# wecacuee/Bayesian_CBF

Hardware: AMD Instinct MI355X
Metric: control steps/sec (GP posterior + CBF-QP) at N_train=512, batch=4096; HBM GB/s vs peak (higher is better)
Workload: dtype f32

## Files before the change

### bayesian_cbf_amd/_lib.py

```python
import ctypes
import os

import torch

_HERE = os.path.dirname(os.path.abspath(__file__))
LIB_PATH = os.environ.get("BCBF_LIB_PATH") or os.path.join(_HERE, "libbcbf.so")

c_int, c_void_p, c_size_t = ctypes.c_int, ctypes.c_void_p, ctypes.c_size_t
c_float, c_double = ctypes.c_float, ctypes.c_double
P = c_void_p

_SIGS = {
    "bcbf_version": (c_int, []),
    "bcbf_last_error": (ctypes.c_char_p, []),
    "bcbf_hbm_read_probe": (c_int, [P, c_size_t, P, ctypes.POINTER(c_size_t), P]),
    "bcbf_lop_elems_f32": (c_size_t, [c_int]),
    "bcbf_lop_elems_f64": (c_size_t, [c_int]),
    "bcbf_posterior_shared_f32": (c_int, [P] * 13 + [c_int, c_int, c_int, c_int, P]),
    "bcbf_posterior_shared_f64": (c_int, [P] * 13 + [c_int, c_int, c_int, c_int, P]),
    "bcbf_posterior_shared_matern52_f32": (c_int, [P] * 13 + [c_int, c_int, c_int, c_int, P]),
    "bcbf_posterior_shared_rbfm52_f32": (c_int, [P] * 13 + [c_int, c_int, c_int, c_int, P]),
    "bcbf_posterior_shared_matern52_f64": (c_int, [P] * 13 + [c_int, c_int, c_int, c_int, P]),
    "bcbf_posterior_shared_rbfm52_f64": (c_int, [P] * 13 + [c_int, c_int, c_int, c_int, P]),
    "bcbf_controller_cones_rows": (c_int, [ctypes.POINTER(c_int), c_int, c_int, c_int]),
    "bcbf_controller_cones_f32": (c_int, [P, P, ctypes.POINTER(c_int), ctypes.POINTER(c_double), c_double, c_double, c_int, c_int, P, P, P, c_int, c_int, c_int, P]),
    "bcbf_controller_cones_f64": (c_int, [P, P, ctypes.POINTER(c_int), ctypes.POINTER(c_double), c_double, c_double, c_int, c_int, P, P, P, c_int, c_int, c_int, P]),
    "bcbf_mll_grad_work_bytes": (c_size_t, [c_int, c_int, c_int]),
    "bcbf_fit_param_count": (c_int, [c_int, c_int, c_int, c_int]),
    "bcbf_coneqp_f64": (c_int, [P, P, P, P, c_int, c_int, ctypes.POINTER(c_int), c_int, P, P, P, c_int, c_int, P]),
    "bcbf_pendulum_control_step_f64": (c_int, [P] * 9 + [c_int] * 4 + [c_double] * 5 + [P, ctypes.POINTER(c_double),
                                               ctypes.POINTER(c_double), c_double, P] + [c_double] * 3 + [c_int] * 2
                                       + [c_double] * 4 + [P] * 24 + [c_int] * 3 + [P] * 3),
    "bcbf_pendulum_control_step_observe_f64": (c_int, [P] * 9 + [c_int] * 4 + [c_double] * 5 + [P, ctypes.POINTER(c_double),
                                                       ctypes.POINTER(c_double), c_double, P] + [c_double] * 3
                                               + [c_int] * 2 + [c_double] * 4 + [P] * 24
                                               + [c_int, P, c_double, ctypes.POINTER(c_double), P, P, P, c_int]
                                               + [c_int] * 3 + [P] * 3),
    "bcbf_pendulum_control_step_sampled_f64": (c_int, [P] * 9 + [c_int] * 4 + [c_double] * 5 + [P, ctypes.POINTER(c_double),
                                                       ctypes.POINTER(c_double), c_double, P] + [c_double] * 3
                                               + [c_int] * 2 + [c_double] * 4 + [P] * 24
                                               + [c_int, P, c_double, ctypes.POINTER(c_double), P, P, P, c_int]
                                               + [P] * 5 + [c_double] + [c_int] * 3 + [P] * 3),
}
_TS_EVENT = [P] * 9 + [c_double] + [P] * 4 + [c_double] * 6 + ["T", P, P, c_double] + [P] * 11
_TS_AUDIT = [P] * 19
_TS_OBSERVE = [c_float, P, P, P, c_int, c_int, c_int, P, c_int]
_TS_SIZES = [c_int] * 5 + [P]
_TSIGS = {
    "bcbf_kb_build": [P, P, P, P, P, P, P, c_int, c_int, c_int, c_int, P],
    "bcbf_kb_build_matern52": [P, P, P, P, P, P, P, c_int, c_int, c_int, c_int, P],
    "bcbf_kb_build_rbfm52": [P, P, P, P, P, P, P, c_int, c_int, c_int, c_int, P],
    "bcbf_posterior_query_matern52": [P] * 13 + [c_int, c_int, c_int, c_int, c_int, P],
    "bcbf_posterior_query_rbfm52": [P] * 13 + [c_int, c_int, c_int, c_int, c_int, P],
    "bcbf_refit": [P, P, P, P, P, P, P, P, P, P, c_int, c_int, c_int, c_int, P],
    "bcbf_refit_retry": [P] * 10 + [c_int, c_int, c_int, c_int, P],
    "bcbf_refit_retry_kind": [P] * 10 + [c_int, c_int, c_int, c_int, c_int, P],
    "bcbf_gram": [P, P, P, c_int, c_int, c_int, c_int, P],
    "bcbf_predict_fullmat": [P] * 17 + [c_int] * 5 + [P],
    "bcbf_unicycle_control_step_observe": [P] * 13 + ["T"] + [P] * 4 + ["T"] + [P] * 16 + ["T", "T", c_int, c_int, c_int, c_int, c_int,
                                           P, P, P, P, c_int, P, c_int, P, P, P],
    "bcbf_unicycle_control_step_sampled": [P] * 13 + ["T"] + [P] * 4 + ["T"] + [P] * 16 + ["T", "T", c_int, c_int, c_int, c_int, c_int,
                                           P, P, P, P, c_int, P, c_int, c_int, P, P, P, P, P, P],
    "bcbf_rollout_risk": [P, P, P, P, P, c_int, c_int, P],
    "bcbf_potrf": [P, P, P, P, c_int, c_int, P],
    "bcbf_subsample_rows": [P, c_int, c_int, c_int, P, P, P, c_int, c_int, c_int, c_int, P, P, P, P, c_int, P],
    "bcbf_trigger_interval": [P] * 8 + [c_double] * 4 + [P, P, P, c_int, c_int, c_int, c_int, P],
    "bcbf_unicycle_trigger_step": _TS_EVENT + _TS_SIZES,
    "bcbf_unicycle_trigger_step_audit": _TS_EVENT + _TS_AUDIT + _TS_SIZES,
    "bcbf_unicycle_trigger_step_observe": _TS_EVENT + _TS_AUDIT + _TS_OBSERVE + _TS_SIZES,
    "bcbf_potrs": [P, P, P, P, P, P, c_int, c_int, c_int, c_int, P],
    "bcbf_chol_append": [P, P, P, P, P, c_int, c_int, P],
    "bcbf_gp_append": [P] * 17 + [c_int, c_int, c_int, c_int, P],
    "bcbf_gp_append_stream": [P] * 20 + [c_int, c_int, c_int, c_int, P],
    "bcbf_gp_reserve": [P] * 8 + [c_int, c_int, c_int, c_int, c_int, c_int, P],
    "bcbf_posterior_query_reserved": [P] * 13 + [c_int, c_int, c_int, c_int, c_int, P],
    "bcbf_gp_append_reserved": [P] * 19 + [c_int, c_int, c_int, c_int, c_int, P],
    "bcbf_gp_append_reserved_raw": [P] * 22 + [c_int, c_int, c_int, c_int, c_int, P],
    "bcbf_gp_tail_step": [P] * 23 + [c_int] * 9 + [P],
    "bcbf_gp_append_stream_kind": [P] * 20 + [c_int, c_int, c_int, c_int, c_int, P],
    "bcbf_posterior_query_reserved_kind": [P] * 13 + [c_int, c_int, c_int, c_int, c_int, c_int, P],
    "bcbf_gp_append_reserved_kind": [P] * 22 + [c_int, c_int, c_int, c_int, c_int, c_int, P],
    "bcbf_gp_tail_step_kind": [P] * 23 + [c_int] * 10 + [P],
    "bcbf_gp_tail_commit": [P, P, P, c_int, c_int, c_int, c_int, c_int, P],
    "bcbf_potri": [P, P, c_int, c_int, P],
    "bcbf_trtri": [P, P, c_int, c_int, P],
    "bcbf_mll_grad": [P] * 16 + [c_int, c_int, c_int, c_int, P, P],
    "bcbf_syrk_lt": [P, P, c_int, c_int, P],
    "bcbf_fit_derive": [P] * 8 + [c_int] * 5 + [P],
    "bcbf_fit_adam_step": [P] * 14 + [c_int] * 7 + [c_double] * 4 + [ctypes.POINTER(c_double), P],
    "bcbf_kinv_apply": [P, P, P, c_int, c_int, c_int, P],
    "bcbf_kb_build_rbflin": [P] * 8 + [c_int, c_int, c_int, c_int, P],
    "bcbf_posterior_query_rbflin": [P] * 14 + [c_int, c_int, c_int, c_int, c_int, P],
    "bcbf_mll_grad_rbflin": [P] * 18 + [c_int, c_int, c_int, c_int, c_int, P, P],
    "bcbf_posterior_step": [P, P, P, P, P, P, P, P, P, P, P, P, c_int, c_int, c_int, c_int, P],
    "bcbf_posterior_query": [P] * 13 + [c_int, c_int, c_int, c_int, c_int, P],
    "bcbf_posterior_jets": [P] * 14 + [c_int, c_int, c_int, c_int, c_int, P],
    "bcbf_cbc2_terms": [P] * 15 + [c_int, c_int, c_int, c_int, c_int, P],
    "bcbf_refit_matern52": [P, P, P, P, P, P, P, P, P, P, c_int, c_int, c_int, c_int, P],
    "bcbf_refit_rbfm52": [P, P, P, P, P, P, P, P, P, P, c_int, c_int, c_int, c_int, P],
    "bcbf_posterior_jets_matern52": [P] * 14 + [c_int, c_int, c_int, c_int, c_int, P],
    "bcbf_posterior_jets_rbfm52": [P] * 14 + [c_int, c_int, c_int, c_int, c_int, P],
    "bcbf_mll_grad_matern52": [P] * 16 + [c_int, c_int, c_int, c_int, P, P],
    "bcbf_mll_grad_rbfm52": [P] * 16 + [c_int, c_int, c_int, c_int, P, P],
    "bcbf_gp_append_matern52": [P] * 17 + [c_int, c_int, c_int, c_int, P],
    "bcbf_gp_append_rbfm52": [P] * 17 + [c_int, c_int, c_int, c_int, P],
    "bcbf_clean_hessian": [P, P, P, c_int, c_int, c_double, c_int, P],
    "bcbf_predict_assemble": [P] * 10 + [c_int] * 5 + [P],
    "bcbf_cbc_terms": [P, P, P, P, P, P, P, P, P, P, P, c_int, c_int, c_int, c_int, P],
    "bcbf_socp": [P, P, P, P, P, P, P, P, c_int, c_int, c_int, c_int, P],
    "bcbf_cbc_socp": [P] * 18 + [c_int, c_int, c_int, c_int, c_int, P],
    "bcbf_unicycle_constraints": [P, P, P, P, "T", P, P, P, P, "T", P, P, P, P, c_int, c_int, P],
    "bcbf_unicycle_step": [P, P, "T", "T", c_int, P],
    "bcbf_pendulum_plant_step": [P, P, "T", "T", "T", "T", c_int, P],
    "bcbf_pendulum_clf_cbf_control": [P, P, c_int, "T", "PT", "T", "T", "T", c_int, "T"] + [P] * 6 + [c_int, P],
    "bcbf_pendulum_clf_cbf_rollout": [P, P, c_int, P, c_int, "T", "PT", "T", "T", "T", c_int, "T", "T"] + [P] * 5
                                     + [c_int] * 4 + [P],
    "bcbf_rollout_stats": [P] * 8 + [c_int, c_int, c_int, P],
    "bcbf_unicycle_control_step": [P] * 13 + ["T"] + [P] * 4 + ["T"] + [P] * 16 + ["T", "T", c_int, c_int, c_int, c_int, c_int, P, P, P],
    "bcbf_unicycle_control_step_matern52": [P] * 13 + ["T"] + [P] * 4 + ["T"] + [P] * 16 + ["T", "T", c_int, c_int, c_int, c_int, c_int, P, P, P],
    "bcbf_unicycle_control_step_rbfm52": [P] * 13 + ["T"] + [P] * 4 + ["T"] + [P] * 16 + ["T", "T", c_int, c_int, c_int, c_int, c_int, P, P, P],
}


def declared_symbols():
    names = list(_SIGS)
    for base in _TSIGS:
        names += [base + "_f32", base + "_f64"]
    return names


def _build_if_missing():
    import fcntl
    with open(os.path.join(_HERE, ".build.lock"), "w") as lock:
        fcntl.flock(lock, fcntl.LOCK_EX)
        try:
            if not os.path.exists(LIB_PATH):
                from . import build as _build
                _build.build()
        finally:
            fcntl.flock(lock, fcntl.LOCK_UN)


def _load():
    if not os.path.exists(LIB_PATH):
        try:
            _build_if_missing()
        except Exception as err:
            raise ImportError(
                "libbcbf.so not found at %s and building it failed (%s) -- build it with "
                "`python -m bayesian_cbf_amd.build` (hipcc, --offload-arch=gfx950).  There is no CPU fallback."
                % (LIB_PATH, err))
    lib = ctypes.CDLL(LIB_PATH)
    for name, (res, args) in _SIGS.items():
        fn = getattr(lib, name)
        fn.restype, fn.argtypes = res, args
    for base, args in _TSIGS.items():
        for suf, ct in (("_f32", c_float), ("_f64", c_double)):
            fn = getattr(lib, base + suf)
            fn.restype = c_int
            fn.argtypes = [ct if a == "T" else ctypes.POINTER(ct) if a == "PT" else a for a in args]
    return lib


lib = _load()


class BcbfError(RuntimeError):
    pass


def check(rc, what):
    if rc != 0:
        msg = lib.bcbf_last_error().decode() if rc == -2 else "invalid argument"
        raise BcbfError("%s failed (rc=%d): %s" % (what, rc, msg))
```

### bayesian_cbf_amd/build.py

```python
import concurrent.futures
import os
import subprocess
import sys

if __package__ in (None, ""):
    sys.path.insert(0, os.path.dirname(os.path.dirname(os.path.abspath(__file__))))
    __package__ = "bayesian_cbf_amd"

HERE = os.path.dirname(os.path.abspath(__file__))
ROOT = os.path.dirname(HERE)
CSRC = os.path.join(HERE, "csrc")
OBJ = os.path.join(HERE, "csrc", "_obj")
LIB = os.path.join(HERE, "libbcbf.so")
ARCH = "gfx950"
SOURCES = ["common.hip", "posterior_step.hip", "jets_mfma.hip", "posterior_shared.hip", "posterior_shared_reg.hip", "refit.hip", "refit_mfma.hip", "refit_mfma64.hip", "refit_wave64.hip", "refit_slab.hip", "solve.hip", "trtri.hip", "tail.hip", "syrk.hip", "mll_grad.hip", "fit.hip", "cbc_terms.hip", "predict_assemble.hip", "gram.hip", "controller_cones.hip", "socp.hip", "socp_quad.hip",
           "unicycle.hip", "control_step.hip", "subsample.hip", "pendulum.hip", "trigger.hip", "trigger_step.hip", "pendulum_qp.hip"]
FLAGS = ["--offload-arch=" + ARCH, "-O3", "-std=c++17", "-fPIC", "-I" + os.path.join(ROOT, "include"),
         "-I" + CSRC, "-Wall", "-Wno-unused-function", "-fvisibility=hidden"]
EXTRA_FLAGS = {"posterior_shared.hip": ["-mllvm", "-amdgpu-mfma-vgpr-form"],
               "refit_wave64.hip": ["-fno-slp-vectorize"],
               "posterior_shared_reg.hip": ["-Rpass-analysis=kernel-resource-usage"],
               "posterior_step.hip": ["-Rpass-analysis=kernel-resource-usage"],
               "pendulum_qp.hip": ["-Rpass-analysis=kernel-resource-usage"],
               "pendulum.hip": ["-Rpass-analysis=kernel-resource-usage"]}
ZERO_SCRATCH_KERNELS = {"posterior_step.hip": [
    "posterior_step_kernel<float, 2, 4, 0, 1, false, 0,", "posterior_step_kernel<float, 3, 4, 0, 1, false, 0,",
    "posterior_step_kernel<double, 2, 4, 0, 1, false, 0,", "posterior_step_kernel<double, 3, 4, 0, 1, false, 0,",
    "posterior_step_kernel<float, 2, 4, 2, 1, false, 0,", "posterior_step_kernel<float, 3, 4, 3, 1, false, 0,",
    "posterior_step_kernel<float, 3, 4, 0, 1, false, 1, false, false>", "posterior_step_kernel<float, 3, 4, 0, 1, true, 0,",
    "posterior_step_kernel<double, 4, 4, 0, 1, false, 0,", "posterior_step_kernel<double, 3, 8, 0, 1, false, 0,"],
    "pendulum_qp.hip": ["pendulum_clf_cbf_rollout_kernel<float>", "pendulum_clf_cbf_rollout_kernel<double>"],
    "pendulum.hip": ["pendulum_sampled_plant_kernel<double>"]}
SCRATCH_ALLOWANCE = {"posterior_step_kernel<float, 3, 4, 3, 1, false, 0,": 40}
NO_SCRATCH = {"posterior_shared_reg.hip"}


def _hipcc():
    for cand in (os.environ.get("HIPCC"), "/opt/rocm/bin/hipcc", "hipcc"):
        if cand and (os.path.sep not in cand or os.path.exists(cand)):
            return cand
    raise RuntimeError("hipcc not found")


def _newer(a, bs):
    if not os.path.exists(a):
        return False
    ta = os.path.getmtime(a)
    return all(os.path.getmtime(b) <= ta for b in bs)


ASAN_FLAGS = ["-O1", "-g", "-fno-omit-frame-pointer", "-fsanitize=address", "-fno-gpu-sanitize", "-shared-libsan"]
ASAN = False


PARTS = {"posterior_shared_reg.hip": dict([("base", ["-DBCBF_PSR_PART_BASE"])] +
                                          [("%s%d" % ("df"[t], c), ["-DBCBF_PSR_PART_T=%d" % t, "-DBCBF_PSR_PART_C=%d" % c])
                                           for t in (0, 1) for c in (2, 3, 4)])}


def _work_list():
    out = []
    for src in SOURCES:
        if src in PARTS and not ASAN:
            out += ["%s#%s" % (src, tag) for tag in PARTS[src]]
        else:
            out.append(src)
    return out


def _compile(item, force):
    src, _, tag = item.partition("#")
    obj = os.path.join(OBJ + ("_asan" if ASAN else ""), os.path.splitext(src)[0] + ("_" + tag if tag else "") + ".o")
    deps = [os.path.join(CSRC, src), os.path.join(ROOT, "include", "bcbf.h"), os.path.abspath(__file__)]
    deps += [os.path.join(CSRC, h) for h in sorted(os.listdir(CSRC)) if h.endswith(".h")]
    if not force and _newer(obj, deps):
        return obj, False
    tuning = os.environ.get("BCBF_EXTRA_HIPCC_FLAGS", "").split()
    flags = [f for f in FLAGS if not (ASAN and f == "-O3")] + (ASAN_FLAGS if ASAN else [])
    extra = list(EXTRA_FLAGS.get(src, [])) + (PARTS[src][tag] if tag else [])
    if ASAN and src == "posterior_shared_reg.hip":
        extra.append("-DBCBF_PSR_DEV")
    cmd = [_hipcc()] + flags + extra + tuning + ["-c", os.path.join(CSRC, src), "-o", obj]
    guard = src in NO_SCRATCH and not ASAN and tag != "base"
    tmpdir = None
    if guard:
        import tempfile
        tmpdir = tempfile.mkdtemp(prefix="bcbf_asm_")
        cmd = cmd[:-1] + [os.path.join(tmpdir, os.path.basename(obj)), "-save-temps=obj"]
    res = subprocess.run(cmd, capture_output=True, text=True)
    if res.returncode != 0:
        raise RuntimeError("hipcc failed for %s:\n%s\n%s" % (src, res.stdout, res.stderr))
    if guard:
        import glob
        import shutil
        from .check_lds_waits import check as _check_lds
        asm = glob.glob(os.path.join(tmpdir, "*-hip-amdgcn-amd-amdhsa-%s.s" % ARCH))
        try:
            if len(asm) != 1:
                raise RuntimeError("%s: no device assembly to check (%s)" % (src, asm))
            bad, checked = _check_lds(open(asm[0]).read(), r"posterior_shared_reg_kernel")
            if bad or not checked:
                raise RuntimeError("%s [%s]: %d instruction(s) touch the destination of an LDS read that is still in flight "
                                   "(explicit ds_read / s_waitcnt pairs; first: %s)" % (src, tag, len(bad), bad[:3]))
            shutil.move(os.path.join(tmpdir, os.path.basename(obj)), obj)
        finally:
            shutil.rmtree(tmpdir, ignore_errors=True)
    if src in ZERO_SCRATCH_KERNELS and not ASAN and not tuning:
        import re
        names = re.findall(r"Function Name: (\S+)", res.stderr)
        sizes = [int(v) for v in re.findall(r"ScratchSize \[bytes/lane\]: (\d+)", res.stderr)]
        dem = subprocess.run(["c++filt"] + names, capture_output=True, text=True).stdout.splitlines() if names else []
        seen = set()
        for full, z in zip(dem, sizes):
            for want in ZERO_SCRATCH_KERNELS[src]:
                if want in full:
                    seen.add(want)
                    if z > SCRATCH_ALLOWANCE.get(want, 0):
                        os.remove(obj)
                        raise RuntimeError("%s: %s uses %d bytes of scratch per lane (its measured figures assume none)" % (src, want, z))
        missing = [w for w in ZERO_SCRATCH_KERNELS[src] if w not in seen]
        if missing or len(names) != len(sizes):
            os.remove(obj)
            raise RuntimeError("%s: the scratch guard found no resource remark for %s" % (src, missing or "the kernels"))
    if guard:
        import re
        names = re.findall(r"Function Name: (\S+)", res.stderr)
        sizes = [int(v) for v in re.findall(r"ScratchSize \[bytes/lane\]: (\d+)", res.stderr)]
        bad = [(n_, z) for n_, z in zip(names, sizes) if z and re.search(r"ELi1ELi\dELi\dEEEv", n_)]
        if not any(re.search(r"ELi1ELi\dELi\dEEEv", n_) for n_ in names) and any("posterior_shared_reg_kernel" in n_ for n_ in names):
            raise RuntimeError("%s: no one-wave-per-SIMD kernel name matched the scratch guard (%s)" % (src, names[:2]))
        if not sizes or len(names) != len(sizes) or bad:
            os.remove(obj)
            raise RuntimeError("%s: kernels with explicit LDS read / wait pairs must not use scratch memory: %s" % (src, bad or "no resource remarks"))
    return obj, True


def build(force=False, verbose=False, asan=False):
    global ASAN
    ASAN = bool(asan)
    try:
        return _build(force, verbose)
    finally:
        ASAN = False


def _build(force, verbose):
    LIB = os.path.join(HERE, "libbcbf_asan.so") if ASAN else globals()["LIB"]
    os.makedirs(OBJ + ("_asan" if ASAN else ""), exist_ok=True)
    work = _work_list()
    with concurrent.futures.ThreadPoolExecutor(max_workers=min(8, len(work))) as ex:
        results = list(ex.map(lambda s: _compile(s, force), work))
    objs = [o for o, _ in results]
    if force or any(changed for _, changed in results) or not _newer(LIB, objs):
        tmp = "%s.tmp.%d" % (LIB, os.getpid())
        cmd = [_hipcc(), "--offload-arch=" + ARCH, "-shared", "-fPIC", "-o", tmp] + objs
        if ASAN:
            cmd += ["-fsanitize=address", "-shared-libsan"]
        res = subprocess.run(cmd, capture_output=True, text=True)
        if res.returncode != 0:
            if os.path.exists(tmp):
                os.remove(tmp)
            raise RuntimeError("link failed:\n%s\n%s" % (res.stdout, res.stderr))
        os.replace(tmp, LIB)
        if verbose:
            print("built", LIB)
    elif verbose:
        print("up to date:", LIB)
    return LIB


if __name__ == "__main__":
    build(force="--force" in sys.argv, verbose=True, asan="--asan" in sys.argv)
```

### bayesian_cbf_amd/csrc/control_step.hip

```cpp
#include "bcbf_common.h"
#include "unicycle_task.h"

namespace bcbf {
template <typename T>
int launch_unicycle_socp(const T* Mk, const T* Bk, const T* A, const T* sign, const T* w, const T* r, const T* relax_mask,
                         const T* rho, T* cones, int* cstatus, T* y, int* status, int* iters, int Bt, int max_iters,
                         const UnicycleTask<T>& task, void* stream);
}

#define BCBF_CTRL(T, SUF, NAME, QUERY, STEP)                                                                           \
    extern "C" int NAME##SUF(                                                                                          \
        const T* Lop, const T* Vw, const T* X, const T* UHB, const T* ell, const T* s2, const T* Bm, const T* M0,     \
        const T* A, T* x, const T* plan, const T* dot_plan, const T* Kp, T clf_gamma, const T* centers,               \
        const T* radii, const T* tw, const T* gammas, T L_mean, const T* w, const T* r, const T* sign,                \
        const T* relax_mask, const T* rho, T* grad, T* cst, T* fhat, T* ghat, T* Mk, T* Bk, T* cones, int* cstatus,   \
        T* y, int* status, int* iters, T dt, T L_true, int Bt, int N, int Kob, int max_iters, int shared_gp,          \
        void* ev_start, void* ev_stop, void* stream) {                                                                 \
        if (Bt <= 0) return BCBF_OK;                                                                                   \
        if (!x || !grad || !cst || !fhat || !ghat || Kob < 0 || Kob + 1 > BCBF_MAX_QUAD_CONSTRAINTS) return BCBF_EINVAL;    \
        hipStream_t st = (hipStream_t)stream;                                                                          \
        if (ev_start) (void)hipEventRecord((hipEvent_t)ev_start, st);                                                  \
            \
        int rc = !Lop ? BCBF_OK : shared_gp ? QUERY##SUF(Lop, Vw, X, UHB, ell, s2, Bm, M0, x, nullptr, Mk, Bk, nullptr, \
                                                        1, Bt, N, 3, 2, stream)                                        \
                           : STEP;                                                                                     \
        if (ev_stop) (void)hipEventRecord((hipEvent_t)ev_stop, st);                                                    \
        if (rc) return rc;                                                                                             \
        bcbf::UnicycleTask<T> task;                                                                                    \
        task.x = x; task.plan = plan; task.dot_plan = dot_plan; task.Kp = Kp; task.centers = centers;                  \
        task.radii = radii; task.tw = tw; task.gammas = gammas; task.clf_gamma = clf_gamma; task.L_mean = L_mean;      \
        task.dt = dt; task.L_true = L_true; task.grad = grad; task.cst = cst; task.fhat = fhat; task.ghat = ghat;      \
        task.Kob = Kob;                                                                                                \
        return bcbf::launch_unicycle_socp<T>(Mk, Bk, A, sign, w, r, relax_mask, rho, cones, cstatus, y, status, iters, \
                                             Bt, max_iters, task, stream);                                             \
    }
#define BCBF_STEP_RBF(SUF) bcbf_posterior_step_##SUF(Lop, Vw, X, UHB, ell, s2, Bm, M0, x, nullptr, Mk, Bk, Bt, N, 3, 2, stream)
#define BCBF_STEP_M52(SUF) bcbf_posterior_query_matern52_##SUF(Lop, Vw, X, UHB, ell, s2, Bm, M0, x, nullptr, Mk, Bk, nullptr, 0, Bt, N, 3, 2, stream)
BCBF_CTRL(float, f32, bcbf_unicycle_control_step_, bcbf_posterior_query_, BCBF_STEP_RBF(f32))
BCBF_CTRL(double, f64, bcbf_unicycle_control_step_, bcbf_posterior_query_, BCBF_STEP_RBF(f64))
BCBF_CTRL(float, f32, bcbf_unicycle_control_step_matern52_, bcbf_posterior_query_matern52_, BCBF_STEP_M52(f32))
BCBF_CTRL(double, f64, bcbf_unicycle_control_step_matern52_, bcbf_posterior_query_matern52_, BCBF_STEP_M52(f64))
#define BCBF_STEP_RM52(SUF) bcbf_posterior_query_rbfm52_##SUF(Lop, Vw, X, UHB, ell, s2, Bm, M0, x, nullptr, Mk, Bk, nullptr, 0, Bt, N, 3, 2, stream)
BCBF_CTRL(float, f32, bcbf_unicycle_control_step_rbfm52_, bcbf_posterior_query_rbfm52_, BCBF_STEP_RM52(f32))
BCBF_CTRL(double, f64, bcbf_unicycle_control_step_rbfm52_, bcbf_posterior_query_rbfm52_, BCBF_STEP_RM52(f64))

#define BCBF_CTRL_OBS(T, SUF)                                                                                          \
    extern "C" int bcbf_unicycle_control_step_observe_##SUF(                                                           \
        const T* Lop, const T* Vw, const T* X, const T* UHB, const T* ell, const T* s2, const T* Bm, const T* M0,     \
        const T* A, T* x, const T* plan, const T* dot_plan, const T* Kp, T clf_gamma, const T* centers,               \
        const T* radii, const T* tw, const T* gammas, T L_mean, const T* w, const T* r, const T* sign,                \
        const T* relax_mask, const T* rho, T* grad, T* cst, T* fhat, T* ghat, T* Mk, T* Bk, T* cones, int* cstatus,   \
        T* y, int* status, int* iters, T dt, T L_true, int Bt, int N, int Kob, int max_iters, int shared_gp,          \
        const T* xq, T* obs_x, T* obs_uh, T* obs_y, int obs_ld, T* xq_next, int flags,                                \
        void* ev_start, void* ev_stop, void* stream) {                                                                 \
        if (Bt <= 0) return BCBF_OK;                                                                                   \
        if (!x || Kob < 0 || Kob + 1 > BCBF_MAX_QUAD_CONSTRAINTS) return BCBF_EINVAL;                                  \
        if ((obs_x || obs_uh || obs_y) && (!obs_x || !obs_uh || !obs_y || obs_ld < 1 || !(dt > T(0)))) return BCBF_EINVAL;   \
        if (grad && (!cst || !fhat || !ghat)) return BCBF_EINVAL;                                                      \
        hipStream_t st = (hipStream_t)stream;                                                                          \
        if (ev_start) (void)hipEventRecord((hipEvent_t)ev_start, st);                                                  \
        const T* q = xq ? xq : x;                                                                                      \
        int rc = !Lop ? BCBF_OK : shared_gp ? bcbf_posterior_query_##SUF(Lop, Vw, X, UHB, ell, s2, Bm, M0, q, nullptr, Mk, Bk, \
                                                                       nullptr, 1, Bt, N, 3, 2, stream)                \
                           : bcbf_posterior_step_##SUF(Lop, Vw, X, UHB, ell, s2, Bm, M0, q, nullptr, Mk, Bk, Bt, N, 3, 2, stream); \
        if (ev_stop) (void)hipEventRecord((hipEvent_t)ev_stop, st);                                                    \
        if (rc) return rc;                                                                                             \
        bcbf::UnicycleTask<T> task;                                                                                    \
        task.x = x; task.plan = plan; task.dot_plan = dot_plan; task.Kp = Kp; task.centers = centers;                  \
        task.radii = radii; task.tw = tw; task.gammas = gammas; task.clf_gamma = clf_gamma; task.L_mean = L_mean;      \
        task.dt = dt; task.L_true = L_true; task.grad = grad; task.cst = cst; task.fhat = fhat; task.ghat = ghat;      \
        task.Kob = Kob; task.obs_x = obs_x; task.obs_uh = obs_uh; task.obs_y = obs_y; task.obs_ld = obs_ld;            \
        task.xq_next = xq_next; task.shift_invariant = flags & 1; task.advance_plan = (flags >> 1) & 1;                \
        return bcbf::launch_unicycle_socp<T>(Mk, Bk, A, sign, w, r, relax_mask, rho, cones, cstatus, y, status, iters, \
                                             Bt, max_iters, task, stream);                                             \
    }
BCBF_CTRL_OBS(float, f32)
BCBF_CTRL_OBS(double, f64)

#define BCBF_CTRL_SAMPLED(T, SUF)                                                                                      \
    extern "C" int bcbf_unicycle_control_step_sampled_##SUF(                                                           \
        const T* Lop, const T* Vw, const T* X, const T* UHB, const T* ell, const T* s2, const T* Bm, const T* M0,     \
        const T* A, T* x, const T* plan, const T* dot_plan, const T* Kp, T clf_gamma, const T* centers,               \
        const T* radii, const T* tw, const T* gammas, T L_mean, const T* w, const T* r, const T* sign,                \
        const T* relax_mask, const T* rho, T* grad, T* cst, T* fhat, T* ghat, T* Mk, T* Bk, T* cones, int* cstatus,   \
        T* y, int* status, int* iters, T dt, T L_true, int Bt, int N, int Kob, int max_iters, int shared_gp,          \
        const T* xq, T* obs_x, T* obs_uh, T* obs_y, int obs_ld, T* xq_next, int flags, int kernel_kind,               \
        const T* z, T* xdot_s, T* cbc_s, void* ev_start, void* ev_stop, void* stream) {                                \
        if (Bt <= 0) return BCBF_OK;                                                                                   \
        if (!x || !z || Kob < 0 || Kob + 1 > BCBF_MAX_QUAD_CONSTRAINTS || kernel_kind < 0 || kernel_kind > 2)          \
            return BCBF_EINVAL;                                                                                        \
        if ((obs_x || obs_uh || obs_y) && (!obs_x || !obs_uh || !obs_y || obs_ld < 1 || !(dt > T(0)))) return BCBF_EINVAL;   \
        if (grad && (!cst || !fhat || !ghat)) return BCBF_EINVAL;                                                      \
        hipStream_t st = (hipStream_t)stream;                                                                          \
        if (ev_start) (void)hipEventRecord((hipEvent_t)ev_start, st);                                                  \
        const T* q = xq ? xq : x;                                                                                      \
        const int sh = shared_gp ? 1 : 0;                                                                              \
        int rc = BCBF_OK;                                                                                              \
        if (Lop && kernel_kind == 1)                                                                                   \
            rc = bcbf_posterior_query_matern52_##SUF(Lop, Vw, X, UHB, ell, s2, Bm, M0, q, nullptr, Mk, Bk, nullptr, sh, Bt, N, 3, 2, stream); \
        else if (Lop && kernel_kind == 2)                                                                              \
            rc = bcbf_posterior_query_rbfm52_##SUF(Lop, Vw, X, UHB, ell, s2, Bm, M0, q, nullptr, Mk, Bk, nullptr, sh, Bt, N, 3, 2, stream); \
        else if (Lop && sh)                                                                                            \
            rc = bcbf_posterior_query_##SUF(Lop, Vw, X, UHB, ell, s2, Bm, M0, q, nullptr, Mk, Bk, nullptr, 1, Bt, N, 3, 2, stream); \
        else if (Lop)                                                                                                  \
            rc = bcbf_posterior_step_##SUF(Lop, Vw, X, UHB, ell, s2, Bm, M0, q, nullptr, Mk, Bk, Bt, N, 3, 2, stream); \
        if (ev_stop) (void)hipEventRecord((hipEvent_t)ev_stop, st);                                                    \
        if (rc) return rc;                                                                                             \
        bcbf::UnicycleTask<T> task;                                                                                    \
        task.x = x; task.plan = plan; task.dot_plan = dot_plan; task.Kp = Kp; task.centers = centers;                  \
        task.radii = radii; task.tw = tw; task.gammas = gammas; task.clf_gamma = clf_gamma; task.L_mean = L_mean;      \
        task.dt = dt; task.L_true = L_true; task.grad = grad; task.cst = cst; task.fhat = fhat; task.ghat = ghat;      \
        task.Kob = Kob; task.obs_x = obs_x; task.obs_uh = obs_uh; task.obs_y = obs_y; task.obs_ld = obs_ld;            \
        task.xq_next = xq_next; task.shift_invariant = flags & 1; task.advance_plan = (flags >> 1) & 1;                \
        task.z = z; task.xdot_s = xdot_s; task.cbc_s = cbc_s;                                                          \
        return bcbf::launch_unicycle_socp<T>(Mk, Bk, A, sign, w, r, relax_mask, rho, cones, cstatus, y, status, iters, \
                                             Bt, max_iters, task, stream);                                             \
    }
BCBF_CTRL_SAMPLED(float, f32)
BCBF_CTRL_SAMPLED(double, f64)
```

### bayesian_cbf_amd/csrc/socp_quad.hip

```cpp
#include "bcbf_common.h"
#include "unicycle_task.h"

namespace bcbf {

template <typename R> struct QTol;
template <> struct QTol<double> {
    static __device__ inline double feas() { return 1e-9; }
    static __device__ inline double gap() { return 1e-9; }
    static __device__ inline double accept() { return 1e-7; }
    static __device__ inline double infeas() { return 1e-8; }
};
__device__ inline float qdv(float a, float b) { return a * __builtin_amdgcn_rcpf(b); }
__device__ inline double qdv(double a, double b) { return a / b; }
__device__ inline float qsq(float a) { return __builtin_amdgcn_sqrtf(a); }
__device__ inline double qsq(double a) { return __builtin_sqrt(a); }

template <int CTRL> __device__ inline float dpp_f(float v) {
    return __builtin_bit_cast(float, __builtin_amdgcn_update_dpp(0, __builtin_bit_cast(int, v), CTRL, 0xF, 0xF, true));
}
template <int CTRL> __device__ inline double dpp_d(double v) {
    const long long b = __builtin_bit_cast(long long, v);
    const int lo = __builtin_amdgcn_update_dpp(0, (int)(b & 0xFFFFFFFFLL), CTRL, 0xF, 0xF, true);
    const int hi = __builtin_amdgcn_update_dpp(0, (int)(b >> 32), CTRL, 0xF, 0xF, true);
    return __builtin_bit_cast(double, ((long long)hi << 32) | (long long)(unsigned)lo);
}
constexpr int QP_XOR1 = 0xB1;
constexpr int QP_XOR2 = 0x4E;
__device__ inline float quad_sum(float v) { v += dpp_f<QP_XOR1>(v); v += dpp_f<QP_XOR2>(v); return v; }
__device__ inline double quad_sum(double v) { v += dpp_d<QP_XOR1>(v); v += dpp_d<QP_XOR2>(v); return v; }
__device__ inline float quad_max(float v) { v = fmaxf(v, dpp_f<QP_XOR1>(v)); v = fmaxf(v, dpp_f<QP_XOR2>(v)); return v; }
__device__ inline double quad_max(double v) { v = fmax(v, dpp_d<QP_XOR1>(v)); v = fmax(v, dpp_d<QP_XOR2>(v)); return v; }

template <typename R, int D>
struct ConeLane {
    R M[D][D], beta2, lam[D], s[D], z[D];

    static __device__ inline R jdet(const R* a) {
        R d = a[0] * a[0];
#pragma unroll
        for (int i = 1; i < D; ++i) d -= a[i] * a[i];
        return d;
    }
    __device__ inline R nt(const R* s_, const R* z_, R* w) {
        R sz = s_[0] * z_[0];
#pragma unroll
        for (int i = 1; i < D; ++i) sz += s_[i] * z_[i];
        const R sn = qsq(jdet(s_)), zn = qsq(jdet(z_));
        const R isn = qdv(R(1), sn), izn = qdv(R(1), zn);
        const R gamma = qsq((R(1) + sz * isn * izn) * R(0.5));
        const R ig = qdv(R(0.5), gamma);
        w[0] = (s_[0] * isn + z_[0] * izn) * ig;
#pragma unroll
        for (int i = 1; i < D; ++i) w[i] = (s_[i] * isn - z_[i] * izn) * ig;
        const R beta = qsq(sn * izn);
        R w1z = 0;
#pragma unroll
        for (int i = 1; i < D; ++i) w1z += w[i] * z_[i];
        lam[0] = beta * (w[0] * z_[0] + w1z);
        const R cf = z_[0] + qdv(w1z, R(1) + w[0]);
#pragma unroll
        for (int i = 1; i < D; ++i) lam[i] = beta * (z_[i] + cf * w[i]);
        return beta;
    }
    __device__ inline void init_scaling() {
        R w[D];
        const R beta = nt(s, z, w);
        beta2 = beta * beta;
        const R iw0 = qdv(R(1), R(1) + w[0]);
#pragma unroll
        for (int a = 0; a < D; ++a)
#pragma unroll
            for (int c = 0; c < D; ++c) {
                R v;
                if (a == 0) v = w[c];
                else if (c == 0) v = w[a];
                else v = (a == c ? R(1) : R(0)) + w[a] * w[c] * iw0;
                M[a][c] = beta * v;
            }
    }
    __device__ inline void minv(const R* v, R* out, R ib2) const {
#pragma unroll
        for (int a = 0; a < D; ++a) {
            R t = 0;
#pragma unroll
            for (int c = 0; c < D; ++c) t += M[c][a] * (c == 0 ? v[c] : -v[c]);
            out[a] = (a == 0 ? t : -t) * ib2;
        }
    }
    __device__ inline void sinv(R* x) const {
        R det = lam[0] * lam[0], lx = 0;
#pragma unroll
        for (int i = 1; i < D; ++i) { det -= lam[i] * lam[i]; lx += lam[i] * x[i]; }
        const R y0 = qdv(lam[0] * x[0] - lx, det);
        const R il0 = qdv(R(1), lam[0]);
        x[0] = y0;
#pragma unroll
        for (int i = 1; i < D; ++i) x[i] = (x[i] - y0 * lam[i]) * il0;
    }
    static __device__ inline void sprod(const R* x, const R* y, R* out) {
        R d = 0;
#pragma unroll
        for (int i = 0; i < D; ++i) d += x[i] * y[i];
        out[0] = d;
#pragma unroll
        for (int i = 1; i < D; ++i) out[i] = x[0] * y[i] + y[0] * x[i];
    }
    __device__ inline R scaled_max_step(const R* x) const {
        const R nrm = qsq(jdet(lam)), inrm = qdv(R(1), nrm);
        const R lb0 = lam[0] * inrm;
        R lx = 0;
#pragma unroll
        for (int i = 1; i < D; ++i) lx += lam[i] * inrm * x[i];
        const R y0 = (lb0 * x[0] - lx) * inrm;
        const R coef = -x[0] + qdv(lx, R(1) + lb0);
        R nn = 0;
#pragma unroll
        for (int i = 1; i < D; ++i) { const R ya = (x[i] + coef * lam[i] * inrm) * inrm; nn += ya * ya; }
        return qsq(nn) - y0;
    }
    __device__ inline void advance(const R* dst, const R* dzt, R step, R ib2) {
#pragma unroll
        for (int a = 0; a < D; ++a) {
            R vs = 0, vz = 0;
#pragma unroll
            for (int c = 0; c < D; ++c) { vs += M[a][c] * dst[c]; vz += M[a][c] * (c == 0 ? dzt[c] : -dzt[c]); }
            s[a] += step * vs;
            z[a] += step * (a == 0 ? vz : -vz) * ib2;
        }
        R st[D], zt[D], w[D];
#pragma unroll
        for (int i = 0; i < D; ++i) { st[i] = lam[i] + step * dst[i]; zt[i] = lam[i] + step * dzt[i]; }
        const R beta = nt(st, zt, w);
        beta2 *= beta * beta;
        const R iw0 = qdv(R(1), R(1) + w[0]);
#pragma unroll
        for (int a = 0; a < D; ++a) {
            const R m0 = M[a][0];
            R mw = 0;
#pragma unroll
            for (int c = 1; c < D; ++c) mw += M[a][c] * w[c];
            const R cf = m0 + mw * iw0;
            M[a][0] = beta * (m0 * w[0] + mw);
#pragma unroll
            for (int c = 1; c < D; ++c) M[a][c] = beta * (M[a][c] + cf * w[c]);
        }
    }
};

__device__ inline double rsqrt_d(double d) {
    double y = __builtin_amdgcn_rsq(d);
    y = y * (1.5 - 0.5 * d * y * y);
    y = y * (1.5 - 0.5 * d * y * y);
    return y;
}
template <int NV>
__device__ inline bool chol3(double (*H)[NV]) {
    bool ok = true;
#pragma unroll
    for (int j = 0; j < NV; ++j) {
        double d = H[j][j];
#pragma unroll
        for (int k = 0; k < NV; ++k) if (k < j) d -= H[j][k] * H[j][k];
        if (!(d > 0.0)) { ok = false; d = 1.0; }
        const double il = rsqrt_d(d);
        H[j][j] = il;
#pragma unroll
        for (int i = 0; i < NV; ++i) if (i > j) {
            double v = H[i][j];
#pragma unroll
            for (int k = 0; k < NV; ++k) if (k < j) v -= H[i][k] * H[j][k];
            H[i][j] = v * il;
        }
    }
    return ok;
}
template <int NV>
__device__ inline void chol3_solve(const double (*H)[NV], double* b) {
#pragma unroll
    for (int i = 0; i < NV; ++i) {
        double v = b[i];
#pragma unroll
        for (int k = 0; k < NV; ++k) if (k < i) v -= H[i][k] * b[k];
        b[i] = v * H[i][i];
    }
#pragma unroll
    for (int ii = 0; ii < NV; ++ii) {
        const int i = NV - 1 - ii;
        double v = b[i];
#pragma unroll
        for (int k = 0; k < NV; ++k) if (k > i) v -= H[k][i] * b[k];
        b[i] = v * H[i][i];
    }
}

template <typename T, bool ON> struct SampledKeep {};
template <typename T> struct SampledKeep<T, true> {
    T x[3], row[3], cst, g[3][2], Mk[9], Bk[9], A[9];
    double sg;
};

template <typename V> __device__ inline V opaque_copy(V v) {
    asm("" : "+v"(v));
    return v;
}

template <typename T, int M_, bool FROM_TERMS, bool UNI, bool SAMPLED = false>
__global__ void __launch_bounds__(64)
socp_quad_kernel(const T* __restrict__ w, const T* __restrict__ r, const T* __restrict__ cones_in,
                 const T* __restrict__ relax_mask, const T* __restrict__ rho,
                 const T* __restrict__ Mk, const T* __restrict__ Bk, const T* __restrict__ A,
                 const T* __restrict__ grad, const T* __restrict__ cst, const T* __restrict__ sign,
                 const T* __restrict__ fhat, const T* __restrict__ ghat, int n,
                 T* __restrict__ terms_out, T* __restrict__ cones_out, int* __restrict__ cstatus,
                 T* __restrict__ y, int* __restrict__ status, int* __restrict__ iters, int Bt, int K, int max_iters,
                 UnicycleTask<T> task) {
    using R = double;
#ifdef BCBF_SOCP_SETPRIO
    __builtin_amdgcn_s_setprio(BCBF_SOCP_SETPRIO);
#endif
    constexpr int NV = M_ + 1, D = M_ + 2, C = M_ + 1;
    constexpr int Q = (M_ + 1) * M_ + (M_ + 1) + M_ + 1;
    constexpr int TW = M_ + 1 + M_ * M_ + M_ + 1;
    const int gid = blockIdx.x * blockDim.x + threadIdx.x;
    const int b = gid >> 2, k = gid & 3;
    const bool inst_ok = b < Bt;
    const int bb = inst_ok ? b : Bt - 1;
    const bool active = k < K;
    const int kk = active ? k : 0;
    [[maybe_unused]] SampledKeep<T, SAMPLED> keep;

    R G[D][NV], h[D];
    const R rh = (R)rho[bb];
    int bad = 0;
    {
        R cA[C][M_], cb[C], cc[M_], cd;
        if (FROM_TERMS) {
            double gd[BCBF_MAX_STATE_DIM];
            double a_h = 0.0, e = 0.0;
            double bfe[M_], Asq[C][C], L[C][C];
            if constexpr (UNI) {
                static_assert(M_ == 2, "unicycle: two controls");
                T xs[3], pl[3], dp[3], kp[3], Mkl[9], Bkl[9], Al[9];
#pragma unroll
                for (int d = 0; d < 3; ++d) {
                    xs[d] = task.x[(size_t)bb * 3 + d];
                    pl[d] = task.plan[(size_t)bb * 3 + d];
                    dp[d] = task.dot_plan[(size_t)bb * 3 + d];
                    kp[d] = task.Kp[d];
                }
#pragma unroll
                for (int a = 0; a < 9; ++a) {
                    Mkl[a] = Mk[(size_t)bb * 9 + a];
                    Bkl[a] = Bk[(size_t)bb * 9 + a];
                    Al[a] = A[(size_t)bb * 9 + a];
                }
                const double sg = (double)sign[kk];
                T cx = T(0), cy = T(0), rad = T(1), gam = T(0), tw0 = T(0), tw1 = T(0);
                if (task.Kob > 0) {
                    const int o = min(max(kk - 1, 0), task.Kob - 1);
                    cx = task.centers[((size_t)bb * task.Kob + o) * 2];
                    cy = task.centers[((size_t)bb * task.Kob + o) * 2 + 1];
                    rad = task.radii[(size_t)bb * task.Kob + o];
                    gam = task.gammas[o];
                    tw0 = task.tw[0];
                    tw1 = task.tw[1];
                }
                T urow[3], ucst = T(0), uG[3][2];
                unicycle_row_vals<T>(kk, xs[0], xs[1], xs[2], pl, dp, kp, task.clf_gamma, cx, cy, rad, tw0, tw1, gam, urow, ucst);
                ackermann_g<T>(xs[2], task.L_mean, uG);
                if constexpr (SAMPLED) {
#pragma unroll
                    for (int d = 0; d < 3; ++d) {
                        keep.x[d] = opaque_copy(xs[d]); keep.row[d] = opaque_copy(urow[d]);
                        keep.g[d][0] = opaque_copy(uG[d][0]); keep.g[d][1] = opaque_copy(uG[d][1]);
                    }
#pragma unroll
                    for (int a = 0; a < 9; ++a) {
                        keep.Mk[a] = opaque_copy(Mkl[a]); keep.Bk[a] = opaque_copy(Bkl[a]); keep.A[a] = opaque_copy(Al[a]);
                    }
                    keep.cst = opaque_copy(ucst);
                    keep.sg = opaque_copy(sg);
                }
#pragma unroll
                for (int d = 0; d < BCBF_MAX_STATE_DIM; ++d) gd[d] = d < 3 ? (double)urow[d < 3 ? d : 0] : 0.0;
                if (inst_ok && active && task.grad != nullptr) {
                    for (int d = 0; d < 3; ++d) task.grad[((size_t)b * K + k) * 3 + d] = urow[d];
                    task.cst[(size_t)b * K + k] = ucst;
                    if (k == 0)
                        for (int d = 0; d < 3; ++d) {
                            task.fhat[(size_t)b * 3 + d] = T(0);
                            task.ghat[((size_t)b * 3 + d) * 2] = uG[d][0];
                            task.ghat[((size_t)b * 3 + d) * 2 + 1] = uG[d][1];
                        }
                }
#pragma unroll
                for (int d = 0; d < 3; ++d) {
                    double t = 0.0;
#pragma unroll
                    for (int e2 = 0; e2 < 3; ++e2) t += (double)Al[d * 3 + e2] * gd[e2];
                    a_h += gd[d] * t;
                }
                e = (double)ucst;
#pragma unroll
                for (int d = 0; d < 3; ++d) e += gd[d] * (double)Mkl[d * 3];
                e *= sg;
#pragma unroll
                for (int i = 0; i < M_; ++i) {
                    double s_ = 0.0;
#pragma unroll
                    for (int d = 0; d < 3; ++d) s_ += ((double)uG[d][i] + (double)Mkl[d * 3 + 1 + i]) * gd[d];
                    bfe[i] = sg * s_;
                }
#pragma unroll
                for (int a = 0; a < C; ++a)
#pragma unroll
                    for (int c = 0; c < C; ++c) { Asq[a][c] = a_h * (double)Bkl[a * 3 + c]; L[a][c] = 0.0; }
            } else {
                const T* Mkb = Mk + (size_t)bb * n * C;
                const T* Bkb = Bk + (size_t)bb * C * C;
                const T* Ab = A + (size_t)bb * n * n;
                const double sg = (double)sign[kk];
                const T* g = grad + ((size_t)bb * K + kk) * n;
#pragma unroll
                for (int d = 0; d < BCBF_MAX_STATE_DIM; ++d) gd[d] = d < n ? (double)g[d] : 0.0;
                for (int d = 0; d < n; ++d) {
                    double t = 0.0;
                    for (int e2 = 0; e2 < n; ++e2) t += (double)Ab[d * n + e2] * gd[e2];
                    a_h += gd[d] * t;
                }
                e = (double)cst[(size_t)bb * K + kk];
                for (int d = 0; d < n; ++d) e += gd[d] * ((double)fhat[(size_t)bb * n + d] + (double)Mkb[d * C]);
                e *= sg;
#pragma unroll
                for (int i = 0; i < M_; ++i) {
                    double s_ = 0.0;
                    for (int d = 0; d < n; ++d)
                        s_ += ((double)ghat[((size_t)bb * n + d) * M_ + i] + (double)Mkb[d * C + 1 + i]) * gd[d];
                    bfe[i] = sg * s_;
                }
#pragma unroll
                for (int a = 0; a < C; ++a)
#pragma unroll
                    for (int c = 0; c < C; ++c) { Asq[a][c] = a_h * (double)Bkb[a * C + c]; L[a][c] = 0.0; }
            }
            if (terms_out && inst_ok && active) {
                T* t = terms_out + ((size_t)b * K + k) * TW;
                for (int i = 0; i < M_; ++i) t[i] = (T)bfe[i];
                t[M_] = (T)e;
                for (int i = 0; i < M_; ++i) for (int j = 0; j < M_; ++j) t[M_ + 1 + i * M_ + j] = (T)Asq[1 + i][1 + j];
                for (int i = 0; i < M_; ++i) t[M_ + 1 + M_ * M_ + i] = (T)(2.0 * Asq[1 + i][0]);
                t[M_ + 1 + M_ * M_ + M_] = (T)Asq[0][0];
            }
#pragma unroll
            for (int j = 0; j < C; ++j) {
                double d = Asq[j][j];
#pragma unroll
                for (int q = 0; q < C; ++q) if (q < j) d -= L[j][q] * L[j][q];
                if (!(d > 0.0)) { bad = BCBF_SOCP_BADCONE; d = 1.0; }
                const double ljj = __builtin_sqrt(d);
                L[j][j] = ljj;
#pragma unroll
                for (int i = 0; i < C; ++i) if (i > j) {
                    double s_ = Asq[i][j];
#pragma unroll
                    for (int q = 0; q < C; ++q) if (q < j) s_ -= L[i][q] * L[j][q];
                    L[i][j] = s_ / ljj;
                }
            }
#pragma unroll
            for (int a = 0; a < C; ++a) {
                cb[a] = (R)L[0][a];
#pragma unroll
                for (int i = 0; i < M_; ++i) cA[a][i] = (R)L[1 + i][a];
            }
#pragma unroll
            for (int i = 0; i < M_; ++i) cc[i] = (R)bfe[i];
            cd = (R)e;
            if (cones_out && inst_ok && active) {
                T* cn = cones_out + ((size_t)b * K + k) * Q;
                for (int a = 0; a < C; ++a) for (int i = 0; i < M_; ++i) cn[a * M_ + i] = (T)cA[a][i];
                for (int a = 0; a < C; ++a) cn[C * M_ + a] = (T)cb[a];
                for (int i = 0; i < M_; ++i) cn[C * M_ + C + i] = (T)cc[i];
                cn[C * M_ + C + M_] = (T)cd;
            }
            if (cstatus && inst_ok && active) cstatus[(size_t)b * K + k] = bad;
        } else {
            const T* cn = cones_in + ((size_t)bb * K + kk) * Q;
#pragma unroll
            for (int a = 0; a < C; ++a) {
                cb[a] = (R)cn[C * M_ + a];
#pragma unroll
                for (int i = 0; i < M_; ++i) cA[a][i] = (R)cn[a * M_ + i];
            }
#pragma unroll
            for (int i = 0; i < M_; ++i) cc[i] = (R)cn[C * M_ + C + i];
            cd = (R)cn[C * M_ + C + M_];
        }
#pragma unroll
        for (int i = 0; i < M_; ++i) G[0][i] = -cc[i];
        G[0][M_] = -(R)relax_mask[kk];
        h[0] = cd;
#pragma unroll
        for (int a = 0; a < C; ++a) {
#pragma unroll
            for (int i = 0; i < M_; ++i) G[1 + a][i] = -rh * cA[a][i];
            G[1 + a][M_] = R(0);
            h[1 + a] = rh * cb[a];
        }
    }
    if (!active) {
#pragma unroll
        for (int a = 0; a < D; ++a) {
            h[a] = a == 0 ? R(1) : R(0);
#pragma unroll
            for (int i = 0; i < NV; ++i) G[a][i] = R(0);
        }
    }
    const bool act = active;
    const bool any_bad = quad_max((R)bad) > R(0);

    R Pd[NV], qv[NV], x[NV];
#pragma unroll
    for (int i = 0; i < NV; ++i) {
        const R wi = (R)w[(size_t)bb * NV + i];
        Pd[i] = R(2) * wi;
        qv[i] = i < M_ ? -R(2) * wi * (R)r[(size_t)bb * M_ + i] : R(0);
    }
    R resx0 = 0, hh = 0;
#pragma unroll
    for (int i = 0; i < NV; ++i) resx0 += qv[i] * qv[i];
#pragma unroll
    for (int a = 0; a < D; ++a) hh += h[a] * h[a];
    hh = active ? hh : R(0);
    resx0 = fmax(R(1), qsq(resx0));
    const R resz0 = fmax(R(1), qsq(quad_sum(hh)));

    ConeLane<R, D> cone;
    double H[NV][NV], rhs[NV];
#pragma unroll
    for (int i = 0; i < NV; ++i) {
        double ri = 0.0;
#pragma unroll
        for (int a = 0; a < D; ++a) ri += (double)G[a][i] * (double)h[a];
        rhs[i] = quad_sum(act ? ri : 0.0) - (double)qv[i];
#pragma unroll
        for (int j = 0; j < NV; ++j) if (j <= i) {
            double v = 0.0;
#pragma unroll
            for (int a = 0; a < D; ++a) v += (double)G[a][i] * (double)G[a][j];
            H[i][j] = quad_sum(act ? v : 0.0) + (i == j ? (double)Pd[i] : 0.0);
        }
    }
    bool okc = chol3<NV>(H);
    chol3_solve<NV>(H, rhs);
#pragma unroll
    for (int i = 0; i < NV; ++i) x[i] = (R)rhs[i];
    {
        R nrm2 = 0;
#pragma unroll
        for (int a = 0; a < D; ++a) {
            R v = -h[a];
#pragma unroll
            for (int i = 0; i < NV; ++i) v += G[a][i] * x[i];
            cone.z[a] = v;
            cone.s[a] = -v;
            nrm2 += v * v;
        }
        const R nrm = fmax(qsq(quad_sum(active ? nrm2 : R(0))), R(1));
        R ns = 0;
#pragma unroll
        for (int a = 1; a < D; ++a) ns += cone.s[a] * cone.s[a];
        ns = qsq(ns);
        const R ts = quad_max(active ? ns - cone.s[0] : R(-1e30));
        const R tz = quad_max(active ? ns - cone.z[0] : R(-1e30));
        if (ts >= R(-1e-8) * nrm) cone.s[0] += R(1) + ts;
        if (tz >= R(-1e-8) * nrm) cone.z[0] += R(1) + tz;
        if (!active) {
#pragma unroll
            for (int a = 0; a < D; ++a) { cone.s[a] = a == 0 ? R(1) : R(0); cone.z[a] = cone.s[a]; }
        }
    }
    cone.init_scaling();

    R xbest[NV], best = R(1e30);
#pragma unroll
    for (int i = 0; i < NV; ++i) xbest[i] = x[i];
    int stall = 0, st_code = BCBF_SOCP_MAXITER, it = 0;
    const R ideg = qdv(R(1), (R)K);
    if (!okc) st_code = BCBF_SOCP_DIVERGED;

    for (it = 0; it <= max_iters && okc; ++it) {
        const R ib2 = qdv(R(1), cone.beta2);
        R gz[NV], rz[D], rzt[D];
#pragma unroll
        for (int i = 0; i < NV; ++i) {
            R t = 0;
#pragma unroll
            for (int a = 0; a < D; ++a) t += G[a][i] * cone.z[a];
            gz[i] = quad_sum(active ? t : R(0));
        }
        R f0 = 0, resx = 0, rz2 = 0, gp = 0;
        R rx[NV];
#pragma unroll
        for (int i = 0; i < NV; ++i) {
            const R px = Pd[i] * x[i];
            f0 += x[i] * (R(0.5) * px + qv[i]);
            rx[i] = px + qv[i] + gz[i];
            resx += rx[i] * rx[i];
        }
#pragma unroll
        for (int a = 0; a < D; ++a) {
            R v = cone.s[a] - h[a];
#pragma unroll
            for (int i = 0; i < NV; ++i) v += G[a][i] * x[i];
            rz[a] = v;
            rz2 += v * v;
            gp += cone.lam[a] * cone.lam[a];
        }
        cone.minv(rz, rzt, ib2);
        R lrz = 0;
#pragma unroll
        for (int a = 0; a < D; ++a) lrz += cone.lam[a] * rzt[a];
        resx = qsq(resx);
        const R resz = qsq(quad_sum(active ? rz2 : R(0)));
        const R gap = quad_sum(active ? gp : R(0));
        lrz = quad_sum(active ? lrz : R(0));
        const R pcost = f0, dcost = f0 + lrz - gap;
        R relgap = R(1e30);
        if (pcost < R(0)) relgap = qdv(gap, -pcost);
        else if (dcost > R(0)) relgap = qdv(gap, dcost);
        const R pres = qdv(resz, resz0), dres = qdv(resx, resx0);
        if (pres <= QTol<R>::feas() && dres <= QTol<R>::feas() && (gap <= QTol<R>::gap() || relgap <= QTol<R>::gap())) {
            st_code = BCBF_SOCP_OPTIMAL;
            break;
        }
        {
            const R merit = fmax(fmax(pres, dres), fmin(gap, relgap));
            stall = merit < R(0.9) * best ? 0 : stall + 1;
            if (merit < best) {
                best = merit;
#pragma unroll
                for (int i = 0; i < NV; ++i) xbest[i] = x[i];
            }
            if (stall >= 3 && best <= QTol<R>::accept()) break;
        }
        {
            R hz = 0, gzn = 0;
#pragma unroll
            for (int a = 0; a < D; ++a) hz += h[a] * cone.z[a];
            hz = quad_sum(active ? hz : R(0));
#pragma unroll
            for (int i = 0; i < NV; ++i) gzn += gz[i] * gz[i];
            if (hz < R(0) && qsq(gzn) <= QTol<R>::infeas() * resx0 * (-hz)) { st_code = BCBF_SOCP_DIVERGED; break; }
        }
        R xmax = 0;
#pragma unroll
        for (int i = 0; i < NV; ++i) xmax = fmax(xmax, fabs(x[i]));
        if (!(gap + resx + resz < R(1e30)) || !(xmax < R(1e12))) { st_code = BCBF_SOCP_DIVERGED; break; }
        if (it == max_iters) break;

        R Gt[D][NV];
#pragma unroll
        for (int i = 0; i < NV; ++i) {
            R col[D], out[D];
#pragma unroll
            for (int a = 0; a < D; ++a) col[a] = G[a][i];
            cone.minv(col, out, ib2);
#pragma unroll
            for (int a = 0; a < D; ++a) Gt[a][i] = out[a];
        }
#pragma unroll
        for (int i = 0; i < NV; ++i)
#pragma unroll
            for (int j = 0; j < NV; ++j) if (j <= i) {
                double v = 0.0;
#pragma unroll
                for (int a = 0; a < D; ++a) v += (double)Gt[a][i] * (double)Gt[a][j];
                H[i][j] = quad_sum(act ? v : 0.0) + (i == j ? (double)Pd[i] : 0.0);
            }
        if (!chol3<NV>(H)) { st_code = BCBF_SOCP_DIVERGED; break; }

        R lsq[D], corr[D], dx[NV], dst[D], dzt[D];
        ConeLane<R, D>::sprod(cone.lam, cone.lam, lsq);
#pragma unroll
        for (int a = 0; a < D; ++a) corr[a] = R(0);
        const R mu = gap * ideg;
        R sigma = R(0), step = R(1);
#pragma unroll
        for (int pass = 0; pass < 2; ++pass) {
            R c[D];
#pragma unroll
            for (int a = 0; a < D; ++a) c[a] = -lsq[a] - corr[a];
            c[0] += sigma * mu;
            cone.sinv(c);
            double rh3[NV];
#pragma unroll
            for (int i = 0; i < NV; ++i) {
                double t = 0.0;
#pragma unroll
                for (int a = 0; a < D; ++a) t += (double)Gt[a][i] * (double)(rzt[a] + c[a]);
                rh3[i] = -(double)rx[i] - quad_sum(act ? t : 0.0);
            }
            chol3_solve<NV>(H, rh3);
#pragma unroll
            for (int i = 0; i < NV; ++i) dx[i] = (R)rh3[i];
#pragma unroll
            for (int a = 0; a < D; ++a) {
                R t = rzt[a];
#pragma unroll
                for (int i = 0; i < NV; ++i) t += Gt[a][i] * dx[i];
                dzt[a] = t + c[a];
                dst[a] = -t;
            }
            R dsdz = 0;
            if (pass == 0) {
                ConeLane<R, D>::sprod(dst, dzt, corr);
#pragma unroll
                for (int a = 0; a < D; ++a) dsdz += dst[a] * dzt[a];
                dsdz = quad_sum(active ? dsdz : R(0));
            }
            const R tloc = active ? fmax(cone.scaled_max_step(dst), cone.scaled_max_step(dzt)) : R(-1e30);
            const R tm = fmax(R(0), quad_max(tloc));
            if (tm == R(0)) step = R(1);
            else step = pass == 0 ? fmin(R(1), qdv(R(1), tm)) : fmin(R(1), qdv(R(0.99), tm));
            if (pass == 0) {
                const R sg = fmin(R(1), fmax(R(0), R(1) - step + qdv(dsdz, gap) * step * step));
                sigma = sg * sg * sg;
            }
        }
#pragma unroll
        for (int i = 0; i < NV; ++i) x[i] += step * dx[i];
        if (active) cone.advance(dst, dzt, step, ib2);
    }
    if (st_code != BCBF_SOCP_OPTIMAL && best <= QTol<R>::accept()) {
#pragma unroll
        for (int i = 0; i < NV; ++i) x[i] = xbest[i];
        st_code = BCBF_SOCP_OPTIMAL;
    }
    if (any_bad) st_code = BCBF_SOCP_BADCONE;
    if (inst_ok && k == 0) {
#pragma unroll
        for (int i = 0; i < NV; ++i) y[(size_t)b * NV + i] = (T)x[i];
        status[b] = st_code;
        if (iters) iters[b] = it;
        if (UNI && !SAMPLED && task.dt > T(0)) {
            T* xs = task.x + (size_t)b * 3;
            const T x0 = xs[0], x1 = xs[1], th = xs[2];
            T n0 = x0, n1 = x1, n2 = th, u0 = T(0), u1 = T(0);
            if (st_code == BCBF_SOCP_OPTIMAL) {
                u0 = (T)x[0]; u1 = (T)x[1];
                ackermann_euler<T>(x0, x1, th, u0, u1, task.dt, task.L_true, n0, n1, n2);
                xs[0] = n0; xs[1] = n1; xs[2] = n2;
            }
            unicycle_observe<T>(task, b, x0, x1, th, n0, n1, n2, u0, u1);
        }
    }
    if constexpr (SAMPLED) {
        static_assert(UNI, "the sampled plant is the unicycle step's");
        if (inst_ok && task.dt > T(0)) {
            const bool solved = st_code == BCBF_SOCP_OPTIMAL;
            double xd[3] = {0.0, 0.0, 0.0}, cb = 0.0;
            T u0 = T(0), u1 = T(0);
            if (solved) {
                u0 = (T)x[0]; u1 = (T)x[1];
                const double ub[3] = {1.0, (double)u0, (double)u1};
                const double rs = __builtin_sqrt(fmax(quad_form3<T>(ub, keep.Bk), 0.0));
                double LA[3][3];
                psd_chol3<T>(keep.A, LA);
                const double z[3] = {(double)task.z[(size_t)b * 3], (double)task.z[(size_t)b * 3 + 1], (double)task.z[(size_t)b * 3 + 2]};
#pragma unroll
                for (int d = 0; d < 3; ++d) {
                    const double gu = (double)keep.g[d][0] * ub[1] + (double)keep.g[d][1] * ub[2];
                    const double mu = (double)keep.Mk[d * 3] + (double)keep.Mk[d * 3 + 1] * ub[1] + (double)keep.Mk[d * 3 + 2] * ub[2];
                    xd[d] = posterior_draw(gu + mu, rs, LA[d], z);
                }
                const double row[3] = {(double)keep.row[0], (double)keep.row[1], (double)keep.row[2]};
                cb = cbc_on(keep.sg, row, xd, (double)keep.cst);
            }
            if (active && task.cbc_s != nullptr) task.cbc_s[(size_t)b * K + k] = (T)cb;
            if (k == 0) {
                T nx[3] = {keep.x[0], keep.x[1], keep.x[2]};
                if (solved) {
#pragma unroll
                    for (int d = 0; d < 3; ++d) {
                        nx[d] = (T)((double)keep.x[d] + xd[d] * (double)task.dt);
                        task.x[(size_t)b * 3 + d] = nx[d];
                    }
                }
                if (task.xdot_s != nullptr)
                    for (int d = 0; d < 3; ++d) task.xdot_s[(size_t)b * 3 + d] = (T)xd[d];
                unicycle_observe<T>(task, b, keep.x[0], keep.x[1], keep.x[2], nx[0], nx[1], nx[2], u0, u1);
            }
        }
    }
}

template <typename T, bool FROM_TERMS>
static int launch_quad(const T* w, const T* r, const T* cones_in, const T* relax_mask, const T* rho, const T* Mk,
                       const T* Bk, const T* A, const T* grad, const T* cst, const T* sign, const T* fhat,
                       const T* ghat, int n, T* terms_out, T* cones_out, int* cstatus, T* y, int* status, int* iters,
                       int Bt, int K, int m, int max_iters, void* stream, const UnicycleTask<T>* task = nullptr) {
    if (Bt <= 0) return BCBF_OK;
    if (!w || !r || !relax_mask || !rho || !y || !status) return BCBF_EINVAL;
    if (K < 1 || K > 4 || m < 1 || m > BCBF_MAX_CTRL_DIM) return BCBF_EINVAL;
    if (FROM_TERMS && task != nullptr) {
        if (!Mk || !Bk || !A || !sign || n != 3 || m != 2 || K != 1 + task->Kob || !task->x || !task->plan ||
            !task->dot_plan || !task->Kp || (task->Kob > 0 && (!task->centers || !task->radii || !task->tw || !task->gammas)))
            return BCBF_EINVAL;
        if (task->grad != nullptr && (!task->cst || !task->fhat || !task->ghat)) return BCBF_EINVAL;
    } else if (FROM_TERMS) {
        if (!Mk || !Bk || !A || !grad || !cst || !sign || !fhat || !ghat || n < 1 || n > BCBF_MAX_STATE_DIM) return BCBF_EINVAL;
    } else if (!cones_in) return BCBF_EINVAL;
    if (max_iters <= 0) max_iters = 100;
    const int threads = 64;
    const long lanes = (long)Bt * 4;
    dim3 grid((unsigned)((lanes + threads - 1) / threads)), block(threads);
    hipStream_t st = (hipStream_t)stream;
    if (FROM_TERMS && task != nullptr && task->z != nullptr) {
        hipLaunchKernelGGL((socp_quad_kernel<T, 2, FROM_TERMS, FROM_TERMS, FROM_TERMS>), grid, block, 0, st, w, r, cones_in,
                           relax_mask, rho, Mk, Bk, A, grad, cst, sign, fhat, ghat, n, terms_out, cones_out, cstatus, y, status,
                           iters, Bt, K, max_iters, *task);
        return check_launch("unicycle_socp_sampled");
    }
    if (FROM_TERMS && task != nullptr) {
        hipLaunchKernelGGL((socp_quad_kernel<T, 2, FROM_TERMS, FROM_TERMS>), grid, block, 0, st, w, r, cones_in, relax_mask,
                           rho, Mk, Bk, A, grad, cst, sign, fhat, ghat, n, terms_out, cones_out, cstatus, y, status, iters,
                           Bt, K, max_iters, *task);
        return check_launch("unicycle_socp");
    }
#define BCBF_Q(MM) hipLaunchKernelGGL((socp_quad_kernel<T, MM, FROM_TERMS, false>), grid, block, 0, st, w, r, cones_in, relax_mask, rho, Mk, Bk, A, grad, cst, sign, fhat, ghat, n, terms_out, cones_out, cstatus, y, status, iters, Bt, K, max_iters, UnicycleTask<T>{})
    switch (m) {
        case 1: BCBF_Q(1); break;
        case 2: BCBF_Q(2); break;
        case 3: BCBF_Q(3); break;
        default: return BCBF_EINVAL;
    }
#undef BCBF_Q
    return check_launch("socp_quad");
}

template <typename T>
int launch_unicycle_socp(const T* Mk, const T* Bk, const T* A, const T* sign, const T* w, const T* r, const T* relax_mask,
                         const T* rho, T* cones, int* cstatus, T* y, int* status, int* iters, int Bt, int max_iters,
                         const UnicycleTask<T>& task, void* stream) {
    return launch_quad<T, true>(w, r, nullptr, relax_mask, rho, Mk, Bk, A, nullptr, nullptr, sign, nullptr, nullptr, 3,
                                nullptr, cones, cstatus, y, status, iters, Bt, 1 + task.Kob, 2, max_iters, stream, &task);
}
template int launch_unicycle_socp<float>(const float*, const float*, const float*, const float*, const float*, const float*,
                                         const float*, const float*, float*, int*, float*, int*, int*, int, int,
                                         const UnicycleTask<float>&, void*);
template int launch_unicycle_socp<double>(const double*, const double*, const double*, const double*, const double*,
                                          const double*, const double*, const double*, double*, int*, double*, int*, int*,
                                          int, int, const UnicycleTask<double>&, void*);

}

extern "C" {
int bcbf_socp_f32(const float* w, const float* r, const float* cones, const float* relax_mask, const float* rho,
                  float* y, int* status, int* iters, int Bt, int K, int m, int max_iters, void* stream) {
    return bcbf::launch_quad<float, false>(w, r, cones, relax_mask, rho, nullptr, nullptr, nullptr, nullptr, nullptr,
                                           nullptr, nullptr, nullptr, 0, nullptr, nullptr, nullptr, y, status, iters,
                                           Bt, K, m, max_iters, stream);
}
int bcbf_socp_f64(const double* w, const double* r, const double* cones, const double* relax_mask, const double* rho,
                  double* y, int* status, int* iters, int Bt, int K, int m, int max_iters, void* stream) {
    return bcbf::launch_quad<double, false>(w, r, cones, relax_mask, rho, nullptr, nullptr, nullptr, nullptr, nullptr,
                                            nullptr, nullptr, nullptr, 0, nullptr, nullptr, nullptr, y, status, iters,
                                            Bt, K, m, max_iters, stream);
}
int bcbf_cbc_socp_f32(const float* Mk, const float* Bk, const float* A, const float* grad, const float* cst,
                      const float* sign, const float* fhat, const float* ghat, const float* w, const float* r,
                      const float* relax_mask, const float* rho, float* terms, float* cones, int* cstatus,
                      float* y, int* status, int* iters, int Bt, int K, int n, int m, int max_iters, void* stream) {
    return bcbf::launch_quad<float, true>(w, r, nullptr, relax_mask, rho, Mk, Bk, A, grad, cst, sign, fhat, ghat, n,
                                          terms, cones, cstatus, y, status, iters, Bt, K, m, max_iters, stream);
}
int bcbf_cbc_socp_f64(const double* Mk, const double* Bk, const double* A, const double* grad, const double* cst,
                      const double* sign, const double* fhat, const double* ghat, const double* w, const double* r,
                      const double* relax_mask, const double* rho, double* terms, double* cones, int* cstatus,
                      double* y, int* status, int* iters, int Bt, int K, int n, int m, int max_iters, void* stream) {
    return bcbf::launch_quad<double, true>(w, r, nullptr, relax_mask, rho, Mk, Bk, A, grad, cst, sign, fhat, ghat, n,
                                           terms, cones, cstatus, y, status, iters, Bt, K, m, max_iters, stream);
}
}
```

### include/bcbf.h

```cpp
#ifndef BCBF_H
#define BCBF_H

#include <stddef.h>
#include <stdint.h>

#ifdef __cplusplus
extern "C" {
#endif
#pragma GCC visibility push(default)

#define BCBF_VERSION_MAJOR 0
#define BCBF_VERSION_MINOR 1

#define BCBF_OK 0
#define BCBF_EINVAL (-1)
#define BCBF_ELAUNCH (-2)

#define BCBF_NB 32
#define BCBF_MAX_STATE_DIM 8
#define BCBF_MAX_CTRL_DIM 3
#define BCBF_MAX_TASK_DIM 12
#define BCBF_MAX_CONSTRAINTS 8
#define BCBF_MAX_QUAD_CONSTRAINTS 4

#define BCBF_SOCP_OPTIMAL 0
#define BCBF_SOCP_MAXITER 1
#define BCBF_SOCP_DIVERGED 2
#define BCBF_SOCP_BADCONE 3

int bcbf_version(void);
const char* bcbf_last_error(void);

int bcbf_hbm_read_probe(const void* buf, size_t bytes, void* sink, size_t* bytes_read, void* stream);

size_t bcbf_lop_elems_f32(int N);
size_t bcbf_lop_elems_f64(int N);

int bcbf_kb_build_f32(const float* X, const float* UH, const float* Bm, const float* ell, const float* s2,
                      const float* jitter, float* Kb, int Bt, int N, int n, int m, void* stream);
int bcbf_kb_build_f64(const double* X, const double* UH, const double* Bm, const double* ell, const double* s2,
                      const double* jitter, double* Kb, int Bt, int N, int n, int m, void* stream);

int bcbf_refit_f32(const float* X, const float* UH, const float* Bm, const float* ell, const float* s2,
                   const float* jitter, float* Lop, float* UHB, float* Ldense, int* info,
                   int Bt, int N, int n, int m, void* stream);
int bcbf_refit_f64(const double* X, const double* UH, const double* Bm, const double* ell, const double* s2,
                   const double* jitter, double* Lop, double* UHB, double* Ldense, int* info,
                   int Bt, int N, int n, int m, void* stream);
int bcbf_refit_retry_f32(const float* X, const float* UH, const float* Bm, const float* ell, const float* s2,
                         const float* jitter, float* Lop, float* UHB, const int* prev_info, int* info,
                         int Bt, int N, int n, int m, void* stream);
int bcbf_refit_retry_f64(const double* X, const double* UH, const double* Bm, const double* ell, const double* s2,
                         const double* jitter, double* Lop, double* UHB, const int* prev_info, int* info,
                         int Bt, int N, int n, int m, void* stream);
int bcbf_refit_retry_kind_f32(const float* X, const float* UH, const float* Bm, const float* ell, const float* s2,
                              const float* jitter, float* Lop, float* UHB, const int* prev_info, int* info,
                              int Bt, int N, int n, int m, int kernel_kind, void* stream);
int bcbf_refit_retry_kind_f64(const double* X, const double* UH, const double* Bm, const double* ell, const double* s2,
                              const double* jitter, double* Lop, double* UHB, const int* prev_info, int* info,
                              int Bt, int N, int n, int m, int kernel_kind, void* stream);

int bcbf_subsample_rows_f32(const float* keys, int ldk, int lo, int P, const float* X, const float* UH, const float* Y,
                            int Ntot, int n, int m, int N, float* Xo, float* UHo, float* Yo, int32_t* idx_out, int B,
                            void* stream);
int bcbf_subsample_rows_f64(const float* keys, int ldk, int lo, int P, const double* X, const double* UH, const double* Y,
                            int Ntot, int n, int m, int N, double* Xo, double* UHo, double* Yo, int32_t* idx_out, int B,
                            void* stream);

int bcbf_trigger_interval_f32(const float* x, const float* off, const float* ls, const float* sf, const float* Adiag,
                              const float* uBu, const float* xvel, const float* Lh, double r, double deltaL, double zeta,
                              double L_alpha, float* Lkd, float* Lfh, float* tau, int B, int Bh, int Nte, int n, void* stream);
int bcbf_trigger_interval_f64(const double* x, const double* off, const double* ls, const double* sf, const double* Adiag,
                              const double* uBu, const double* xvel, const double* Lh, double r, double deltaL, double zeta,
                              double L_alpha, double* Lkd, double* Lfh, double* tau, int B, int Bh, int Nte, int n, void* stream);

int bcbf_unicycle_trigger_step_f32(float* x, const float* y, const int* status, const float* fhat, const float* ghat, const float* Mk,
                                   const float* centers, const float* tw, const float* off, double r, const float* ls, const float* sf,
                                   const float* Adiag, const float* Bhyp, double deltaL, double zeta, double L_alpha, double tau_min,
                                   double tau_max, double t_end, float L_true, const float* plan_all, const float* dplan_all,
                                   double dt_plan, double* t, int* events, float* plan, float* dot_plan, float* tau, float* dt_used,
                                   float* Lfh, float* Lkd, float* Lh, float* xvel, float* uBu, int Bt, int Bh, int Kob, int Nte, int P,
                                   void* stream);
int bcbf_unicycle_trigger_step_f64(double* x, const double* y, const int* status, const double* fhat, const double* ghat,
                                   const double* Mk, const double* centers, const double* tw, const double* off, double r,
                                   const double* ls, const double* sf, const double* Adiag, const double* Bhyp, double deltaL, double zeta,
                                   double L_alpha, double tau_min, double tau_max, double t_end, double L_true, const double* plan_all,
                                   const double* dplan_all, double dt_plan, double* t, int* events, double* plan, double* dot_plan,
                                   double* tau, double* dt_used, double* Lfh, double* Lkd, double* Lh, double* xvel, double* uBu, int Bt,
                                   int Bh, int Kob, int Nte, int P, void* stream);

int bcbf_unicycle_trigger_step_audit_f32(float* x, const float* y, const int* status, const float* fhat, const float* ghat,
                                         const float* Mk, const float* centers, const float* tw, const float* off, double r,
                                         const float* ls, const float* sf, const float* Adiag, const float* Bhyp, double deltaL,
                                         double zeta, double L_alpha, double tau_min, double tau_max, double t_end, float L_true,
                                         const float* plan_all, const float* dplan_all, double dt_plan, double* t, int* events,
                                         float* plan, float* dot_plan, float* tau, float* dt_used, float* Lfh, float* Lkd, float* Lh,
                                         float* xvel, float* uBu, const float* Bk, const float* A, const float* grad,
                                         const float* cst, const float* sign, const float* rho, const float* z, float* xdot_s,
                                         float* cbc_s, int* viol, int* solved, float* min_cbc, float* u_held, int* held,
                                         float* held_mean, float* held_margin, int* audit_n, int* audit_neg, float* audit_min, int Bt,
                                         int Bh, int Kob, int Nte, int P, void* stream);
int bcbf_unicycle_trigger_step_audit_f64(double* x, const double* y, const int* status, const double* fhat, const double* ghat,
                                         const double* Mk, const double* centers, const double* tw, const double* off, double r,
                                         const double* ls, const double* sf, const double* Adiag, const double* Bhyp, double deltaL,
                                         double zeta, double L_alpha, double tau_min, double tau_max, double t_end, double L_true,
                                         const double* plan_all, const double* dplan_all, double dt_plan, double* t, int* events,
                                         double* plan, double* dot_plan, double* tau, double* dt_used, double* Lfh, double* Lkd,
                                         double* Lh, double* xvel, double* uBu, const double* Bk, const double* A, const double* grad,
                                         const double* cst, const double* sign, const double* rho, const double* z, double* xdot_s,
                                         double* cbc_s, int* viol, int* solved, double* min_cbc, double* u_held, int* held,
                                         double* held_mean, double* held_margin, int* audit_n, int* audit_neg, double* audit_min,
                                         int Bt, int Bh, int Kob, int Nte, int P, void* stream);

int bcbf_unicycle_trigger_step_observe_f32(float* x, const float* y, const int* status, const float* fhat, const float* ghat,
        const float* Mk, const float* centers, const float* tw, const float* off, double r, const float* ls, const float* sf, const float* Adiag,
        const float* Bhyp, double deltaL, double zeta, double L_alpha, double tau_min, double tau_max, double t_end, float L_true,
        const float* plan_all, const float* dplan_all, double dt_plan, double* t, int* events, float* plan, float* dot_plan, float* tau,
        float* dt_used, float* Lfh, float* Lkd, float* Lh, float* xvel, float* uBu, const float* Bk, const float* A, const float* grad, const float* cst,
        const float* sign, const float* rho, const float* z, float* xdot_s, float* cbc_s, int* viol, int* solved, float* min_cbc, float* u_held,
        int* held, float* held_mean, float* held_margin, int* audit_n, int* audit_neg, float* audit_min, float L_mean, float* obs_x,
        float* obs_uh, float* obs_y, int obs_ld, int obs_row0, int obs_every, float* xq_next, int flags, int Bt, int Bh, int Kob, int Nte,
        int P, void* stream);
int bcbf_unicycle_trigger_step_observe_f64(double* x, const double* y, const int* status, const double* fhat, const double* ghat,
        const double* Mk, const double* centers, const double* tw, const double* off, double r, const double* ls, const double* sf, const double* Adiag,
        const double* Bhyp, double deltaL, double zeta, double L_alpha, double tau_min, double tau_max, double t_end, double L_true,
        const double* plan_all, const double* dplan_all, double dt_plan, double* t, int* events, double* plan, double* dot_plan, double* tau,
        double* dt_used, double* Lfh, double* Lkd, double* Lh, double* xvel, double* uBu, const double* Bk, const double* A, const double* grad, const double* cst,
        const double* sign, const double* rho, const double* z, double* xdot_s, double* cbc_s, int* viol, int* solved, double* min_cbc, double* u_held,
        int* held, double* held_mean, double* held_margin, int* audit_n, int* audit_neg, double* audit_min, float L_mean, double* obs_x,
        double* obs_uh, double* obs_y, int obs_ld, int obs_row0, int obs_every, double* xq_next, int flags, int Bt, int Bh, int Kob, int Nte,
        int P, void* stream);

int bcbf_potrf_f32(const float* Kb, float* Lop, float* Ldense, int* info, int Bt, int N, void* stream);
int bcbf_potrf_f64(const double* Kb, double* Lop, double* Ldense, int* info, int Bt, int N, void* stream);

int bcbf_potrs_f32(const float* Lop, const float* Xdot, const float* UH, const float* M0,
                   float* Vw, float* alpha, int Bt, int N, int n, int m, void* stream);
int bcbf_potrs_f64(const double* Lop, const double* Xdot, const double* UH, const double* M0,
                   double* Vw, double* alpha, int Bt, int N, int n, int m, void* stream);

int bcbf_chol_append_f32(const float* Lop_in, const float* knew, const float* kappa, float* Lop_out,
                         int* info, int Bt, int N, void* stream);
int bcbf_chol_append_f64(const double* Lop_in, const double* knew, const double* kappa, double* Lop_out,
                         int* info, int Bt, int N, void* stream);

int bcbf_gp_append_f32(const float* Lop_in, const float* Vw_in, const float* X_in, const float* UHB_in,
                       const float* ell, const float* s2, const float* Bm, const float* M0, const float* x_new,
                       const float* uh_new, const float* xdot_new, const float* jitter_new, float* Lop_out,
                       float* Vw_out, float* X_out, float* UHB_out, int* info, int Bt, int N, int n, int m, void* stream);
int bcbf_gp_append_f64(const double* Lop_in, const double* Vw_in, const double* X_in, const double* UHB_in,
                       const double* ell, const double* s2, const double* Bm, const double* M0, const double* x_new,
                       const double* uh_new, const double* xdot_new, const double* jitter_new, double* Lop_out,
                       double* Vw_out, double* X_out, double* UHB_out, int* info, int Bt, int N, int n, int m,
                       void* stream);
int bcbf_gp_append_stream_f32(const float* Lop_in, const float* Vw_in, const float* X_in, const float* UHB_in,
                              const float* ell, const float* s2, const float* Bm, const float* M0, const float* x_new,
                              const float* uh_new, const float* xdot_new, const float* jitter_new, float* Lop_out,
                              float* Vw_out, float* X_out, float* UHB_out, int* info, float* Wwork, float* Mk_work,
                              float* Bk_work, int Bt, int N, int n, int m, void* stream);
int bcbf_gp_append_stream_f64(const double* Lop_in, const double* Vw_in, const double* X_in, const double* UHB_in,
                              const double* ell, const double* s2, const double* Bm, const double* M0, const double* x_new,
                              const double* uh_new, const double* xdot_new, const double* jitter_new, double* Lop_out,
                              double* Vw_out, double* X_out, double* UHB_out, int* info, double* Wwork, double* Mk_work,
                              double* Bk_work, int Bt, int N, int n, int m, void* stream);

int bcbf_refit_matern52_f32(const float* X, const float* UH, const float* Bm, const float* ell, const float* s2,
                            const float* jitter, float* Lop, float* UHB, float* Ldense, int* info, int Bt, int N, int n, int m,
                            void* stream);
int bcbf_refit_matern52_f64(const double* X, const double* UH, const double* Bm, const double* ell, const double* s2,
                            const double* jitter, double* Lop, double* UHB, double* Ldense, int* info, int Bt, int N, int n, int m,
                            void* stream);
int bcbf_posterior_jets_matern52_f32(const float* Lop, const float* Vw, const float* X, const float* UHB,
                                     const float* ell, const float* s2, const float* Bm, const float* M0,
                                     const float* xq, float* Mk, float* Bk, float* G, float* Mj, float* Wj, int shared,
                                     int Bt, int N, int n, int m, void* stream);
int bcbf_posterior_jets_matern52_f64(const double* Lop, const double* Vw, const double* X, const double* UHB,
                                     const double* ell, const double* s2, const double* Bm, const double* M0,
                                     const double* xq, double* Mk, double* Bk, double* G, double* Mj, double* Wj, int shared,
                                     int Bt, int N, int n, int m, void* stream);
int bcbf_mll_grad_matern52_f32(const float* Lop, const float* alpha, const float* Kinv, const float* X, const float* UH,
                               const float* R, const float* Ainv, const float* Bm, const float* ell, const float* s2, float* g_ell,
                               float* g_s2, float* g_B, float* logdetK, float* RtA, float* UHtA, int Bt, int N, int n, int m,
                               void* work, void* stream);
int bcbf_mll_grad_matern52_f64(const double* Lop, const double* alpha, const double* Kinv, const double* X, const double* UH,
                               const double* R, const double* Ainv, const double* Bm, const double* ell, const double* s2,
                               double* g_ell, double* g_s2, double* g_B, double* logdetK, double* RtA, double* UHtA, int Bt, int N,
                               int n, int m, void* work, void* stream);
int bcbf_gp_append_matern52_f32(const float* Lop_in, const float* Vw_in, const float* X_in, const float* UHB_in,
                                const float* ell, const float* s2, const float* Bm, const float* M0, const float* x_new,
                                const float* uh_new, const float* xdot_new, const float* jitter_new, float* Lop_out,
                                float* Vw_out, float* X_out, float* UHB_out, int* info, int Bt, int N, int n, int m, void* stream);
int bcbf_gp_append_matern52_f64(const double* Lop_in, const double* Vw_in, const double* X_in, const double* UHB_in,
                                const double* ell, const double* s2, const double* Bm, const double* M0, const double* x_new,
                                const double* uh_new, const double* xdot_new, const double* jitter_new, double* Lop_out,
                                double* Vw_out, double* X_out, double* UHB_out, int* info, int Bt, int N, int n, int m,
                                void* stream);
int bcbf_kb_build_matern52_f32(const float* X, const float* UH, const float* Bm, const float* ell, const float* s2,
                               const float* jitter, float* Kb, int Bt, int N, int n, int m, void* stream);
int bcbf_kb_build_matern52_f64(const double* X, const double* UH, const double* Bm, const double* ell, const double* s2,
                               const double* jitter, double* Kb, int Bt, int N, int n, int m, void* stream);
int bcbf_posterior_query_matern52_f32(const float* Lop, const float* Vw, const float* X, const float* UHB,
                                      const float* ell, const float* s2, const float* Bm, const float* M0, const float* xq,
                                      const float* jitter2, float* Mk, float* Bk, float* W, int shared, int Bt, int N,
                                      int n, int m, void* stream);
int bcbf_posterior_query_matern52_f64(const double* Lop, const double* Vw, const double* X, const double* UHB,
                                      const double* ell, const double* s2, const double* Bm, const double* M0,
                                      const double* xq, const double* jitter2, double* Mk, double* Bk, double* W,
                                      int shared, int Bt, int N, int n, int m, void* stream);

int bcbf_rollout_stats_f32(const float* cst, const float* y, const int* status, const float* w, const float* gammas,
                           float* min_h, float* cost, int* fails, int Bt, int Kob, int nv, void* stream);
int bcbf_rollout_stats_f64(const double* cst, const double* y, const int* status, const double* w, const double* gammas,
                           double* min_h, double* cost, int* fails, int Bt, int Kob, int nv, void* stream);
int bcbf_rollout_risk_f32(const float* cbc_s, const int* status, int* viol, int* solved, float* min_cbc, int Bt, int Kob,
                          void* stream);
int bcbf_rollout_risk_f64(const double* cbc_s, const int* status, int* viol, int* solved, double* min_cbc, int Bt, int Kob,
                          void* stream);

int bcbf_gp_reserve_f32(const float* Lop_in, const float* Vw_in, const float* X_in, const float* UHB_in, float* Lop_r,
                        float* Vw_r, float* X_r, float* UHB_r, int Bt, int N, int Ncap_in, int Ncap, int n, int m,
                        void* stream);
int bcbf_gp_reserve_f64(const double* Lop_in, const double* Vw_in, const double* X_in, const double* UHB_in, double* Lop_r,
                        double* Vw_r, double* X_r, double* UHB_r, int Bt, int N, int Ncap_in, int Ncap, int n, int m,
                        void* stream);
int bcbf_posterior_query_reserved_f32(const float* Lop_r, const float* Vw_r, const float* X_r, const float* UHB_r,
                                      const float* ell, const float* s2, const float* Bm, const float* M0, const float* xq,
                                      const float* jitter2, float* Mk, float* Bk, float* W, int Bt, int N, int Ncap, int n,
                                      int m, void* stream);
int bcbf_posterior_query_reserved_f64(const double* Lop_r, const double* Vw_r, const double* X_r, const double* UHB_r,
                                      const double* ell, const double* s2, const double* Bm, const double* M0,
                                      const double* xq, const double* jitter2, double* Mk, double* Bk, double* W, int Bt,
                                      int N, int Ncap, int n, int m, void* stream);
int bcbf_gp_append_reserved_f32(float* Lop_r, float* Vw_r, float* X_r, float* UHB_r, const float* ell, const float* s2,
                                const float* Bm, const float* M0, const float* x_new, const float* uh_new,
                                const float* xdot_new, const float* jitter_new, int* info, float* Wwork, float* Mk_work,
                                float* Bk_work, const float* xq, float* Mk, float* Bk, int Bt, int N, int Ncap, int n, int m,
                                void* stream);
int bcbf_gp_append_reserved_f64(double* Lop_r, double* Vw_r, double* X_r, double* UHB_r, const double* ell, const double* s2,
                                const double* Bm, const double* M0, const double* x_new, const double* uh_new,
                                const double* xdot_new, const double* jitter_new, int* info, double* Wwork, double* Mk_work,
                                double* Bk_work, const double* xq, double* Mk, double* Bk, int Bt, int N, int Ncap, int n,
                                int m, void* stream);
int bcbf_gp_append_reserved_raw_f32(float* Lop_r, float* Vw_r, float* X_r, float* UHB_r, const float* ell, const float* s2,
                                    const float* Bm, const float* M0, const float* x_new, const float* uh_new,
                                    const float* xdot_new, const float* jitter_new, int* info, float* Wwork, float* Mk_work,
                                    float* Bk_work, const float* xq, float* Mk, float* Bk, float* rawUH, float* rawY,
                                    float* rawJ, int Bt, int N, int Ncap, int n, int m, void* stream);
int bcbf_gp_append_reserved_raw_f64(double* Lop_r, double* Vw_r, double* X_r, double* UHB_r, const double* ell,
                                    const double* s2, const double* Bm, const double* M0, const double* x_new,
                                    const double* uh_new, const double* xdot_new, const double* jitter_new, int* info,
                                    double* Wwork, double* Mk_work, double* Bk_work, const double* xq, double* Mk, double* Bk,
                                    double* rawUH, double* rawY, double* rawJ, int Bt, int N, int Ncap, int n, int m,
                                    void* stream);

int bcbf_gp_tail_step_f32(const float* Lop_r, float* Vw_r, float* X_r, float* UHB_r, const float* ell, const float* s2,
                          const float* Bm, const float* M0, const float* xq, const float* x_new, const float* uh_new,
                          const float* xdot_new, const float* jitter_new, float* Rb, float* Rinv, int* info, float* Wwork,
                          float* swork, float* Mk, float* Bk, float* rawUH, float* rawY, float* rawJ, int Bt, int N0, int t,
                          int tcap, int Ncap, int Lcap, int n, int m, int do_append, void* stream);
int bcbf_gp_tail_step_f64(const double* Lop_r, double* Vw_r, double* X_r, double* UHB_r, const double* ell, const double* s2,
                          const double* Bm, const double* M0, const double* xq, const double* x_new, const double* uh_new,
                          const double* xdot_new, const double* jitter_new, double* Rb, double* Rinv, int* info, double* Wwork,
                          double* swork, double* Mk, double* Bk, double* rawUH, double* rawY, double* rawJ, int Bt, int N0, int t,
                          int tcap, int Ncap, int Lcap, int n, int m, int do_append, void* stream);

int bcbf_gp_tail_commit_f32(float* Lop_r, const float* Rb, const float* Rinv, int Bt, int N0, int t, int tcap, int Ncap, void* stream);
int bcbf_gp_tail_commit_f64(double* Lop_r, const double* Rb, const double* Rinv, int Bt, int N0, int t, int tcap, int Ncap, void* stream);

int bcbf_gp_append_stream_kind_f32(const float* Lop_in, const float* Vw_in, const float* X_in, const float* UHB_in,
                                   const float* ell, const float* s2, const float* Bm, const float* M0, const float* x_new,
                                   const float* uh_new, const float* xdot_new, const float* jitter_new, float* Lop_out,
                                   float* Vw_out, float* X_out, float* UHB_out, int* info, float* Wwork, float* Mk_work,
                                   float* Bk_work, int Bt, int N, int n, int m, int kernel_kind, void* stream);
int bcbf_gp_append_stream_kind_f64(const double* Lop_in, const double* Vw_in, const double* X_in, const double* UHB_in,
                                   const double* ell, const double* s2, const double* Bm, const double* M0,
                                   const double* x_new, const double* uh_new, const double* xdot_new,
                                   const double* jitter_new, double* Lop_out, double* Vw_out, double* X_out, double* UHB_out,
                                   int* info, double* Wwork, double* Mk_work, double* Bk_work, int Bt, int N, int n, int m,
                                   int kernel_kind, void* stream);
int bcbf_posterior_query_reserved_kind_f32(const float* Lop_r, const float* Vw_r, const float* X_r, const float* UHB_r,
                                           const float* ell, const float* s2, const float* Bm, const float* M0,
                                           const float* xq, const float* jitter2, float* Mk, float* Bk, float* W, int Bt,
                                           int N, int Ncap, int n, int m, int kernel_kind, void* stream);
int bcbf_posterior_query_reserved_kind_f64(const double* Lop_r, const double* Vw_r, const double* X_r, const double* UHB_r,
                                           const double* ell, const double* s2, const double* Bm, const double* M0,
                                           const double* xq, const double* jitter2, double* Mk, double* Bk, double* W, int Bt,
                                           int N, int Ncap, int n, int m, int kernel_kind, void* stream);
int bcbf_gp_append_reserved_kind_f32(float* Lop_r, float* Vw_r, float* X_r, float* UHB_r, const float* ell, const float* s2,
                                     const float* Bm, const float* M0, const float* x_new, const float* uh_new,
                                     const float* xdot_new, const float* jitter_new, int* info, float* Wwork, float* Mk_work,
                                     float* Bk_work, const float* xq, float* Mk, float* Bk, float* rawUH, float* rawY,
                                     float* rawJ, int Bt, int N, int Ncap, int n, int m, int kernel_kind, void* stream);
int bcbf_gp_append_reserved_kind_f64(double* Lop_r, double* Vw_r, double* X_r, double* UHB_r, const double* ell,
                                     const double* s2, const double* Bm, const double* M0, const double* x_new,
                                     const double* uh_new, const double* xdot_new, const double* jitter_new, int* info,
                                     double* Wwork, double* Mk_work, double* Bk_work, const double* xq, double* Mk, double* Bk,
                                     double* rawUH, double* rawY, double* rawJ, int Bt, int N, int Ncap, int n, int m,
                                     int kernel_kind, void* stream);
int bcbf_gp_tail_step_kind_f32(const float* Lop_r, float* Vw_r, float* X_r, float* UHB_r, const float* ell, const float* s2,
                               const float* Bm, const float* M0, const float* xq, const float* x_new, const float* uh_new,
                               const float* xdot_new, const float* jitter_new, float* Rb, float* Rinv, int* info,
                               float* Wwork, float* swork, float* Mk, float* Bk, float* rawUH, float* rawY, float* rawJ, int Bt,
                               int N0, int t, int tcap, int Ncap, int Lcap, int n, int m, int do_append, int kernel_kind,
                               void* stream);
int bcbf_gp_tail_step_kind_f64(const double* Lop_r, double* Vw_r, double* X_r, double* UHB_r, const double* ell,
                               const double* s2, const double* Bm, const double* M0, const double* xq, const double* x_new,
                               const double* uh_new, const double* xdot_new, const double* jitter_new, double* Rb,
                               double* Rinv, int* info, double* Wwork, double* swork, double* Mk, double* Bk, double* rawUH,
                               double* rawY, double* rawJ, int Bt, int N0, int t, int tcap, int Ncap, int Lcap, int n, int m,
                               int do_append, int kernel_kind, void* stream);

int bcbf_potri_f32(const float* Lop, float* Kinv, int Bt, int N, void* stream);
int bcbf_potri_f64(const double* Lop, double* Kinv, int Bt, int N, void* stream);
int bcbf_trtri_f32(const float* Lop, float* Linv, int Bt, int N, void* stream);
int bcbf_trtri_f64(const double* Lop, double* Linv, int Bt, int N, void* stream);
int bcbf_syrk_lt_f32(const float* Linv, float* Kinv, int Bt, int N, void* stream);
int bcbf_syrk_lt_f64(const double* Linv, double* Kinv, int Bt, int N, void* stream);

size_t bcbf_mll_grad_work_bytes(int Bt, int N, int m);
int bcbf_mll_grad_f32(const float* Lop, const float* alpha, const float* Kinv, const float* X, const float* UH,
                      const float* R, const float* Ainv, const float* Bm, const float* ell, const float* s2, float* g_ell,
                      float* g_s2, float* g_B, float* logdetK, float* RtA, float* UHtA, int Bt, int N, int n, int m,
                      void* work, void* stream);
int bcbf_mll_grad_f64(const double* Lop, const double* alpha, const double* Kinv, const double* X, const double* UH,
                      const double* R, const double* Ainv, const double* Bm, const double* ell, const double* s2,
                      double* g_ell, double* g_s2, double* g_B, double* logdetK, double* RtA, double* UHtA, int Bt, int N,
                      int n, int m, void* work, void* stream);

int bcbf_fit_param_count(int n, int m, int rA, int rB);
int bcbf_fit_derive_f32(const float* theta, float* ell, float* s2, float* A, float* Bm, float* M0, float* Ainv, float* logdetA,
                        int Bt, int n, int m, int rA, int rB, void* stream);
int bcbf_fit_derive_f64(const double* theta, double* ell, double* s2, double* A, double* Bm, double* M0, double* Ainv,
                        double* logdetA, int Bt, int n, int m, int rA, int rB, void* stream);
int bcbf_fit_adam_step_f32(float* theta, float* mom1, float* mom2, const float* g_ell, const float* g_s2, const float* g_B,
                           const float* logdetK, const float* RtA, const float* UHtA, const float* Ainv, const float* logdetA,
                           const int* skip, float* loss, float* grad_out, int Bt, int N, int n, int m, int rA, int rB, int step,
                           double lr, double beta1, double beta2, double eps, const double* gamma_prior, void* stream);
int bcbf_fit_adam_step_f64(double* theta, double* mom1, double* mom2, const double* g_ell, const double* g_s2, const double* g_B,
                           const double* logdetK, const double* RtA, const double* UHtA, const double* Ainv, const double* logdetA,
                           const int* skip, double* loss, double* grad_out, int Bt, int N, int n, int m, int rA, int rB, int step,
                           double lr, double beta1, double beta2, double eps, const double* gamma_prior, void* stream);
int bcbf_kinv_apply_f32(const float* Kinv, const float* R, float* alpha, int Bt, int N, int nt, void* stream);
int bcbf_kinv_apply_f64(const double* Kinv, const double* R, double* alpha, int Bt, int N, int nt, void* stream);

int bcbf_posterior_step_f32(const float* Lop, const float* Vw, const float* X, const float* UHB,
                            const float* ell, const float* s2, const float* Bm, const float* M0,
                            const float* xq, const float* jitter2, float* Mk, float* Bk,
                            int Bt, int N, int n, int m, void* stream);
int bcbf_posterior_step_f64(const double* Lop, const double* Vw, const double* X, const double* UHB,
                            const double* ell, const double* s2, const double* Bm, const double* M0,
                            const double* xq, const double* jitter2, double* Mk, double* Bk,
                            int Bt, int N, int n, int m, void* stream);

int bcbf_posterior_query_f32(const float* Lop, const float* Vw, const float* X, const float* UHB,
                             const float* ell, const float* s2, const float* Bm, const float* M0,
                             const float* xq, const float* jitter2, float* Mk, float* Bk, float* W,
                             int shared, int Bt, int N, int n, int m, void* stream);
int bcbf_posterior_query_f64(const double* Lop, const double* Vw, const double* X, const double* UHB,
                             const double* ell, const double* s2, const double* Bm, const double* M0,
                             const double* xq, const double* jitter2, double* Mk, double* Bk, double* W,
                             int shared, int Bt, int N, int n, int m, void* stream);

int bcbf_posterior_shared_f32(const float* Lop, const float* Vw, const float* X, const float* UHB,
                              const float* ell, const float* s2, const float* Bm, const float* M0,
                              const float* xq, const float* jitter2, float* Mk, float* Bk, float* W,
                              int Bt, int N, int n, int m, void* stream);
int bcbf_posterior_shared_f64(const double* Lop, const double* Vw, const double* X, const double* UHB,
                              const double* ell, const double* s2, const double* Bm, const double* M0,
                              const double* xq, const double* jitter2, double* Mk, double* Bk, double* W,
                              int Bt, int N, int n, int m, void* stream);
int bcbf_posterior_shared_matern52_f32(const float* Lop, const float* Vw, const float* X, const float* UHB,
                                       const float* ell, const float* s2, const float* Bm, const float* M0,
                                       const float* xq, const float* jitter2, float* Mk, float* Bk, float* W,
                                       int Bt, int N, int n, int m, void* stream);
int bcbf_posterior_shared_matern52_f64(const double* Lop, const double* Vw, const double* X, const double* UHB,
                                       const double* ell, const double* s2, const double* Bm, const double* M0,
                                       const double* xq, const double* jitter2, double* Mk, double* Bk, double* W,
                                       int Bt, int N, int n, int m, void* stream);

int bcbf_predict_assemble_f32(const float* G, const float* Xq, const float* Xqp, const float* ell, const float* s2,
                              const float* Bm, const float* A, const float* jitter, float* BkXX, float* Kron, int b, int bp,
                              int n, int m, int kernel_kind, void* stream);
int bcbf_predict_assemble_f64(const double* G, const double* Xq, const double* Xqp, const double* ell, const double* s2,
                              const double* Bm, const double* A, const double* jitter, double* BkXX, double* Kron, int b, int bp,
                              int n, int m, int kernel_kind, void* stream);

int bcbf_gram_f32(const float* W, const float* Wp, float* G, int b, int bp, int Np, int C, void* stream);
int bcbf_gram_f64(const double* W, const double* Wp, double* G, int b, int bp, int Np, int C, void* stream);
int bcbf_predict_fullmat_f32(const float* Lop, const float* Vw, const float* X, const float* UHB, const float* ell,
                             const float* s2, const float* Bm, const float* M0, const float* A, const float* Xq,
                             const float* jitter, float* Mk, float* Bk, float* W, float* G, float* BkXX, float* Kron, int b,
                             int N, int n, int m, int kernel_kind, void* stream);
int bcbf_predict_fullmat_f64(const double* Lop, const double* Vw, const double* X, const double* UHB, const double* ell,
                             const double* s2, const double* Bm, const double* M0, const double* A, const double* Xq,
                             const double* jitter, double* Mk, double* Bk, double* W, double* G, double* BkXX, double* Kron,
                             int b, int N, int n, int m, int kernel_kind, void* stream);

int bcbf_posterior_jets_f32(const float* Lop, const float* Vw, const float* X, const float* UHB,
                            const float* ell, const float* s2, const float* Bm, const float* M0,
                            const float* xq, float* Mk, float* Bk, float* G, float* Mj, float* Wj, int shared,
                            int Bt, int N, int n, int m, void* stream);
int bcbf_posterior_jets_f64(const double* Lop, const double* Vw, const double* X, const double* UHB,
                            const double* ell, const double* s2, const double* Bm, const double* M0,
                            const double* xq, double* Mk, double* Bk, double* G, double* Mj, double* Wj, int shared,
                            int Bt, int N, int n, int m, void* stream);

int bcbf_cbc2_terms_f32(const float* Mk, const float* Bk, const float* G, const float* Mj, const float* A,
                        const float* Bm, const float* ell, const float* s2, const float* h, const float* gh,
                        const float* Hh, const float* kalpha, const float* u0, float* out, int* status,
                        int Bt, int n, int m, int hessian_mode, int kernel_kind, void* stream);
int bcbf_cbc2_terms_f64(const double* Mk, const double* Bk, const double* G, const double* Mj, const double* A,
                        const double* Bm, const double* ell, const double* s2, const double* h, const double* gh,
                        const double* Hh, const double* kalpha, const double* u0, double* out, int* status,
                        int Bt, int n, int m, int hessian_mode, int kernel_kind, void* stream);

int bcbf_clean_hessian_f32(const float* Hin, float* Hout, int* status, int Bt, int n, double eps, int mode, void* stream);
int bcbf_clean_hessian_f64(const double* Hin, double* Hout, int* status, int Bt, int n, double eps, int mode, void* stream);

int bcbf_cbc_terms_f32(const float* Mk, const float* Bk, const float* A, const float* grad, const float* cst,
                       const float* sign, const float* fhat, const float* ghat,
                       float* terms, float* cones, int* cstatus, int Bt, int K, int n, int m, void* stream);
int bcbf_cbc_terms_f64(const double* Mk, const double* Bk, const double* A, const double* grad, const double* cst,
                       const double* sign, const double* fhat, const double* ghat,
                       double* terms, double* cones, int* cstatus, int Bt, int K, int n, int m, void* stream);

int bcbf_socp_f32(const float* w, const float* r, const float* cones, const float* relax_mask, const float* rho,
                  float* y, int* status, int* iters, int Bt, int K, int m, int max_iters, void* stream);
int bcbf_socp_f64(const double* w, const double* r, const double* cones, const double* relax_mask, const double* rho,
                  double* y, int* status, int* iters, int Bt, int K, int m, int max_iters, void* stream);

int bcbf_cbc_socp_f32(const float* Mk, const float* Bk, const float* A, const float* grad, const float* cst,
                      const float* sign, const float* fhat, const float* ghat, const float* w, const float* r,
                      const float* relax_mask, const float* rho, float* terms, float* cones, int* cstatus,
                      float* y, int* status, int* iters, int Bt, int K, int n, int m, int max_iters, void* stream);
int bcbf_cbc_socp_f64(const double* Mk, const double* Bk, const double* A, const double* grad, const double* cst,
                      const double* sign, const double* fhat, const double* ghat, const double* w, const double* r,
                      const double* relax_mask, const double* rho, double* terms, double* cones, int* cstatus,
                      double* y, int* status, int* iters, int Bt, int K, int n, int m, int max_iters, void* stream);

int bcbf_coneqp_f64(const double* P, const double* q, const double* G, const double* h,
                    int nv, int l, const int* qdims, int nq,
                    double* x, int* status, int* iters, int Bt, int max_iters, void* stream);

int bcbf_kb_build_rbflin_f32(const float* X, const float* UH, const float* Bm, const float* ell, const float* s2,
                             const float* lin, const float* jitter, float* Kb, int Bt, int N, int n, int m, void* stream);
int bcbf_kb_build_rbflin_f64(const double* X, const double* UH, const double* Bm, const double* ell, const double* s2,
                             const double* lin, const double* jitter, double* Kb, int Bt, int N, int n, int m,
                             void* stream);
int bcbf_posterior_query_rbflin_f32(const float* Lop, const float* Vw, const float* X, const float* UHB,
                                    const float* ell, const float* s2, const float* lin, const float* Bm,
                                    const float* M0, const float* xq, const float* jitter2, float* Mk,
                                    float* Bk, float* W, int shared, int Bt, int N, int n, int m, void* stream);
int bcbf_posterior_query_rbflin_f64(const double* Lop, const double* Vw, const double* X, const double* UHB,
                                    const double* ell, const double* s2, const double* lin, const double* Bm,
                                    const double* M0, const double* xq, const double* jitter2, double* Mk,
                                    double* Bk, double* W, int shared, int Bt, int N, int n, int m, void* stream);
int bcbf_mll_grad_rbflin_f32(const float* Lop, const float* alpha, const float* Kinv, const float* X, const float* UH,
                             const float* R, const float* Ainv, const float* Bm, const float* ell, const float* s2,
                             const float* lin, float* g_ell, float* g_s2, float* g_lin, float* g_B, float* logdetK,
                             float* RtA, float* UHtA, int Bt, int N, int n, int m, int nt, void* work, void* stream);
int bcbf_mll_grad_rbflin_f64(const double* Lop, const double* alpha, const double* Kinv, const double* X,
                             const double* UH, const double* R, const double* Ainv, const double* Bm, const double* ell,
                             const double* s2, const double* lin, double* g_ell, double* g_s2, double* g_lin,
                             double* g_B, double* logdetK, double* RtA, double* UHtA, int Bt, int N, int n, int m,
                             int nt, void* work, void* stream);

int bcbf_controller_cones_rows(const int* kind, int K, int m, int objective);
int bcbf_controller_cones_f32(const float* terms, const float* u_ref, const int* kind, const double* factor,
                              double ctrl_reg, double relax_weight, int extravars, int objective, double* G, double* h,
                              int* cstatus, int Bt, int K, int m, void* stream);
int bcbf_controller_cones_f64(const double* terms, const double* u_ref, const int* kind, const double* factor,
                              double ctrl_reg, double relax_weight, int extravars, int objective, double* G, double* h,
                              int* cstatus, int Bt, int K, int m, void* stream);

int bcbf_unicycle_constraints_f32(const float* x, const float* plan, const float* dot_plan, const float* Kp,
                                  float clf_gamma, const float* centers, const float* radii, const float* tw,
                                  const float* gammas, float L_mean, float* grad, float* cst, float* fhat,
                                  float* ghat, int Bt, int Kob, void* stream);
int bcbf_unicycle_constraints_f64(const double* x, const double* plan, const double* dot_plan, const double* Kp,
                                  double clf_gamma, const double* centers, const double* radii, const double* tw,
                                  const double* gammas, double L_mean, double* grad, double* cst, double* fhat,
                                  double* ghat, int Bt, int Kob, void* stream);

int bcbf_unicycle_step_f32(float* x, const float* u, float dt, float L_true, int Bt, void* stream);
int bcbf_unicycle_step_f64(double* x, const double* u, double dt, double L_true, int Bt, void* stream);

int bcbf_unicycle_control_step_f32(
    const float* Lop, const float* Vw, const float* X, const float* UHB, const float* ell, const float* s2,
    const float* Bm, const float* M0, const float* A, float* x, const float* plan, const float* dot_plan,
    const float* Kp, float clf_gamma, const float* centers, const float* radii, const float* tw, const float* gammas,
    float L_mean, const float* w, const float* r, const float* sign, const float* relax_mask, const float* rho,
    float* grad, float* cst, float* fhat, float* ghat, float* Mk, float* Bk, float* cones, int* cstatus,
    float* y, int* status, int* iters, float dt, float L_true, int Bt, int N, int Kob, int max_iters, int shared_gp,
    void* ev_start, void* ev_stop, void* stream);
int bcbf_unicycle_control_step_f64(
    const double* Lop, const double* Vw, const double* X, const double* UHB, const double* ell, const double* s2,
    const double* Bm, const double* M0, const double* A, double* x, const double* plan, const double* dot_plan,
    const double* Kp, double clf_gamma, const double* centers, const double* radii, const double* tw,
    const double* gammas, double L_mean, const double* w, const double* r, const double* sign,
    const double* relax_mask, const double* rho, double* grad, double* cst, double* fhat, double* ghat, double* Mk,
    double* Bk, double* cones, int* cstatus, double* y, int* status, int* iters, double dt, double L_true, int Bt,
    int N, int Kob, int max_iters, int shared_gp, void* ev_start, void* ev_stop, void* stream);
int bcbf_unicycle_control_step_observe_f32(
    const float* Lop, const float* Vw, const float* X, const float* UHB, const float* ell, const float* s2,
    const float* Bm, const float* M0, const float* A, float* x, const float* plan, const float* dot_plan,
    const float* Kp, float clf_gamma, const float* centers, const float* radii, const float* tw, const float* gammas,
    float L_mean, const float* w, const float* r, const float* sign, const float* relax_mask, const float* rho,
    float* grad, float* cst, float* fhat, float* ghat, float* Mk, float* Bk, float* cones, int* cstatus,
    float* y, int* status, int* iters, float dt, float L_true, int Bt, int N, int Kob, int max_iters, int shared_gp,
    const float* xq, float* obs_x, float* obs_uh, float* obs_y, int obs_ld, float* xq_next, int flags,
    void* ev_start, void* ev_stop, void* stream);
int bcbf_unicycle_control_step_observe_f64(
    const double* Lop, const double* Vw, const double* X, const double* UHB, const double* ell, const double* s2,
    const double* Bm, const double* M0, const double* A, double* x, const double* plan, const double* dot_plan,
    const double* Kp, double clf_gamma, const double* centers, const double* radii, const double* tw,
    const double* gammas, double L_mean, const double* w, const double* r, const double* sign,
    const double* relax_mask, const double* rho, double* grad, double* cst, double* fhat, double* ghat, double* Mk,
    double* Bk, double* cones, int* cstatus, double* y, int* status, int* iters, double dt, double L_true, int Bt,
    int N, int Kob, int max_iters, int shared_gp, const double* xq, double* obs_x, double* obs_uh, double* obs_y,
    int obs_ld, double* xq_next, int flags, void* ev_start, void* ev_stop, void* stream);
int bcbf_unicycle_control_step_sampled_f32(
    const float* Lop, const float* Vw, const float* X, const float* UHB, const float* ell, const float* s2,
    const float* Bm, const float* M0, const float* A, float* x, const float* plan, const float* dot_plan,
    const float* Kp, float clf_gamma, const float* centers, const float* radii, const float* tw, const float* gammas,
    float L_mean, const float* w, const float* r, const float* sign, const float* relax_mask, const float* rho,
    float* grad, float* cst, float* fhat, float* ghat, float* Mk, float* Bk, float* cones, int* cstatus,
    float* y, int* status, int* iters, float dt, float L_true, int Bt, int N, int Kob, int max_iters, int shared_gp,
    const float* xq, float* obs_x, float* obs_uh, float* obs_y, int obs_ld, float* xq_next, int flags, int kernel_kind,
    const float* z, float* xdot_s, float* cbc_s, void* ev_start, void* ev_stop, void* stream);
int bcbf_unicycle_control_step_sampled_f64(
    const double* Lop, const double* Vw, const double* X, const double* UHB, const double* ell, const double* s2,
    const double* Bm, const double* M0, const double* A, double* x, const double* plan, const double* dot_plan,
    const double* Kp, double clf_gamma, const double* centers, const double* radii, const double* tw,
    const double* gammas, double L_mean, const double* w, const double* r, const double* sign,
    const double* relax_mask, const double* rho, double* grad, double* cst, double* fhat, double* ghat, double* Mk,
    double* Bk, double* cones, int* cstatus, double* y, int* status, int* iters, double dt, double L_true, int Bt,
    int N, int Kob, int max_iters, int shared_gp, const double* xq, double* obs_x, double* obs_uh, double* obs_y,
    int obs_ld, double* xq_next, int flags, int kernel_kind, const double* z, double* xdot_s, double* cbc_s,
    void* ev_start, void* ev_stop, void* stream);

int bcbf_pendulum_plant_step_f32(float* x, const float* u, float mass, float gravity, float length, float dt, int Bt,
                                 void* stream);
int bcbf_pendulum_plant_step_f64(double* x, const double* u, double mass, double gravity, double length, double dt,
                                 int Bt, void* stream);

#define BCBF_PENDULUM_BADHESSIAN 5

int bcbf_pendulum_control_step_f64(
    const double* Lop, const double* Vw, const double* X, const double* UHB, const double* ell, const double* s2,
    const double* Bm, const double* M0, const double* A, int N, int shared, int kernel_kind,
    int mean_model, double mean_mass, double mean_gravity, double mean_length,
    double theta_c, double delta_c, const double* kalpha, const double* x_goal, const double* Q_goal, double R,
    const double* u_ref_in, double safety_factor, double ctrl_reg, double relax_weight, int hessian_mode, int max_iters,
    double true_mass, double true_gravity, double true_length, double dt,
    double* x, double* Mk, double* Bk, double* G, double* Mj, double* h, double* gh, double* Hh, double* u_ref,
    double* terms2, double* terms, int* tstatus, double* Gc, double* hc, int* cstatus, double* P, double* q,
    double* y, int* sstatus, int* iters, double* u, int* status, double* min_h, int* fails,
    int Bt, int n, int m, void* ev_start, void* ev_stop, void* stream);

int bcbf_pendulum_control_step_observe_f64(
    const double* Lop, const double* Vw, const double* X, const double* UHB, const double* ell, const double* s2,
    const double* Bm, const double* M0, const double* A, int N, int shared, int kernel_kind,
    int mean_model, double mean_mass, double mean_gravity, double mean_length,
    double theta_c, double delta_c, const double* kalpha, const double* x_goal, const double* Q_goal, double R,
    const double* u_ref_in, double safety_factor, double ctrl_reg, double relax_weight, int hessian_mode, int max_iters,
    double true_mass, double true_gravity, double true_length, double dt,
    double* x, double* Mk, double* Bk, double* G, double* Mj, double* h, double* gh, double* Hh, double* u_ref,
    double* terms2, double* terms, int* tstatus, double* Gc, double* hc, int* cstatus, double* P, double* q,
    double* y, int* sstatus, int* iters, double* u, int* status, double* min_h, int* fails,
    int prior, const double* explore, double eps, const double* ctrl_range, double* obs_x, double* obs_uh, double* obs_y,
    int obs_ld, int Bt, int n, int m, void* ev_start, void* ev_stop, void* stream);

int bcbf_pendulum_control_step_sampled_f64(
    const double* Lop, const double* Vw, const double* X, const double* UHB, const double* ell, const double* s2,
    const double* Bm, const double* M0, const double* A, int N, int shared, int kernel_kind,
    int mean_model, double mean_mass, double mean_gravity, double mean_length,
    double theta_c, double delta_c, const double* kalpha, const double* x_goal, const double* Q_goal, double R,
    const double* u_ref_in, double safety_factor, double ctrl_reg, double relax_weight, int hessian_mode, int max_iters,
    double true_mass, double true_gravity, double true_length, double dt,
    double* x, double* Mk, double* Bk, double* G, double* Mj, double* h, double* gh, double* Hh, double* u_ref,
    double* terms2, double* terms, int* tstatus, double* Gc, double* hc, int* cstatus, double* P, double* q,
    double* y, int* sstatus, int* iters, double* u, int* status, double* min_h, int* fails,
    int prior, const double* explore, double eps, const double* ctrl_range, double* obs_x, double* obs_uh, double* obs_y,
    int obs_ld, const double* z, double* xdot_s, double* cbc_s, int* relaxed, int* viol_relaxed, double rho_tol,
    int Bt, int n, int m, void* ev_start, void* ev_stop, void* stream);

int bcbf_pendulum_clf_cbf_control_f32(const float* x, const float* ctrl_params, int ctrl_stride, float clf_c,
                                      const float* k_alpha, float theta_c, float delta_c, float cbf_gamma, int cbf_kind,
                                      float slack_weight, float* A, float* b, float* values, float* u, float* rho,
                                      int* status, int Bt, void* stream);
int bcbf_pendulum_clf_cbf_control_f64(const double* x, const double* ctrl_params, int ctrl_stride, double clf_c,
                                      const double* k_alpha, double theta_c, double delta_c, double cbf_gamma, int cbf_kind,
                                      double slack_weight, double* A, double* b, double* values, double* u, double* rho,
                                      int* status, int Bt, void* stream);

int bcbf_pendulum_clf_cbf_rollout_f32(float* x, const float* ctrl_params, int ctrl_stride, const float* true_params,
                                      int true_stride, float clf_c, const float* k_alpha, float theta_c, float delta_c,
                                      float cbf_gamma, int cbf_kind, float slack_weight, float dt, float* min_h, int* damage,
                                      int* status, float* traj, float* u_rec, int record_every, int t_offset, int numSteps,
                                      int Bt, void* stream);
int bcbf_pendulum_clf_cbf_rollout_f64(double* x, const double* ctrl_params, int ctrl_stride, const double* true_params,
                                      int true_stride, double clf_c, const double* k_alpha, double theta_c, double delta_c,
                                      double cbf_gamma, int cbf_kind, double slack_weight, double dt, double* min_h,
                                      int* damage, int* status, double* traj, double* u_rec, int record_every, int t_offset,
                                      int numSteps, int Bt, void* stream);
int bcbf_unicycle_control_step_matern52_f32(
    const float* Lop, const float* Vw, const float* X, const float* UHB, const float* ell, const float* s2,
    const float* Bm, const float* M0, const float* A, float* x, const float* plan, const float* dot_plan,
    const float* Kp, float clf_gamma, const float* centers, const float* radii, const float* tw, const float* gammas,
    float L_mean, const float* w, const float* r, const float* sign, const float* relax_mask, const float* rho,
    float* grad, float* cst, float* fhat, float* ghat, float* Mk, float* Bk, float* cones, int* cstatus,
    float* y, int* status, int* iters, float dt, float L_true, int Bt, int N, int Kob, int max_iters, int shared_gp,
    void* ev_start, void* ev_stop, void* stream);
int bcbf_unicycle_control_step_matern52_f64(
    const double* Lop, const double* Vw, const double* X, const double* UHB, const double* ell, const double* s2,
    const double* Bm, const double* M0, const double* A, double* x, const double* plan, const double* dot_plan,
    const double* Kp, double clf_gamma, const double* centers, const double* radii, const double* tw,
    const double* gammas, double L_mean, const double* w, const double* r, const double* sign,
    const double* relax_mask, const double* rho, double* grad, double* cst, double* fhat, double* ghat, double* Mk,
    double* Bk, double* cones, int* cstatus, double* y, int* status, int* iters, double dt, double L_true, int Bt,
    int N, int Kob, int max_iters, int shared_gp, void* ev_start, void* ev_stop, void* stream);

int bcbf_refit_rbfm52_f32(const float* X, const float* UH, const float* Bm, const float* ell, const float* s2,
                            const float* jitter, float* Lop, float* UHB, float* Ldense, int* info, int Bt, int N, int n, int m,
                            void* stream);
int bcbf_refit_rbfm52_f64(const double* X, const double* UH, const double* Bm, const double* ell, const double* s2,
                            const double* jitter, double* Lop, double* UHB, double* Ldense, int* info, int Bt, int N, int n, int m,
                            void* stream);
int bcbf_posterior_jets_rbfm52_f32(const float* Lop, const float* Vw, const float* X, const float* UHB,
                                     const float* ell, const float* s2, const float* Bm, const float* M0,
                                     const float* xq, float* Mk, float* Bk, float* G, float* Mj, float* Wj, int shared,
                                     int Bt, int N, int n, int m, void* stream);
int bcbf_posterior_jets_rbfm52_f64(const double* Lop, const double* Vw, const double* X, const double* UHB,
                                     const double* ell, const double* s2, const double* Bm, const double* M0,
                                     const double* xq, double* Mk, double* Bk, double* G, double* Mj, double* Wj, int shared,
                                     int Bt, int N, int n, int m, void* stream);
int bcbf_mll_grad_rbfm52_f32(const float* Lop, const float* alpha, const float* Kinv, const float* X, const float* UH,
                               const float* R, const float* Ainv, const float* Bm, const float* ell, const float* s2, float* g_ell,
                               float* g_s2, float* g_B, float* logdetK, float* RtA, float* UHtA, int Bt, int N, int n, int m,
                               void* work, void* stream);
int bcbf_mll_grad_rbfm52_f64(const double* Lop, const double* alpha, const double* Kinv, const double* X, const double* UH,
                               const double* R, const double* Ainv, const double* Bm, const double* ell, const double* s2,
                               double* g_ell, double* g_s2, double* g_B, double* logdetK, double* RtA, double* UHtA, int Bt, int N,
                               int n, int m, void* work, void* stream);
int bcbf_gp_append_rbfm52_f32(const float* Lop_in, const float* Vw_in, const float* X_in, const float* UHB_in,
                                const float* ell, const float* s2, const float* Bm, const float* M0, const float* x_new,
                                const float* uh_new, const float* xdot_new, const float* jitter_new, float* Lop_out,
                                float* Vw_out, float* X_out, float* UHB_out, int* info, int Bt, int N, int n, int m, void* stream);
int bcbf_gp_append_rbfm52_f64(const double* Lop_in, const double* Vw_in, const double* X_in, const double* UHB_in,
                                const double* ell, const double* s2, const double* Bm, const double* M0, const double* x_new,
                                const double* uh_new, const double* xdot_new, const double* jitter_new, double* Lop_out,
                                double* Vw_out, double* X_out, double* UHB_out, int* info, int Bt, int N, int n, int m,
                                void* stream);
int bcbf_kb_build_rbfm52_f32(const float* X, const float* UH, const float* Bm, const float* ell, const float* s2,
                               const float* jitter, float* Kb, int Bt, int N, int n, int m, void* stream);
int bcbf_kb_build_rbfm52_f64(const double* X, const double* UH, const double* Bm, const double* ell, const double* s2,
                               const double* jitter, double* Kb, int Bt, int N, int n, int m, void* stream);
int bcbf_posterior_query_rbfm52_f32(const float* Lop, const float* Vw, const float* X, const float* UHB,
                                      const float* ell, const float* s2, const float* Bm, const float* M0, const float* xq,
                                      const float* jitter2, float* Mk, float* Bk, float* W, int shared, int Bt, int N,
                                      int n, int m, void* stream);
int bcbf_posterior_query_rbfm52_f64(const double* Lop, const double* Vw, const double* X, const double* UHB,
                                      const double* ell, const double* s2, const double* Bm, const double* M0,
                                      const double* xq, const double* jitter2, double* Mk, double* Bk, double* W,
                                      int shared, int Bt, int N, int n, int m, void* stream);
int bcbf_posterior_shared_rbfm52_f32(const float* Lop, const float* Vw, const float* X, const float* UHB,
                                       const float* ell, const float* s2, const float* Bm, const float* M0,
                                       const float* xq, const float* jitter2, float* Mk, float* Bk, float* W,
                                       int Bt, int N, int n, int m, void* stream);
int bcbf_posterior_shared_rbfm52_f64(const double* Lop, const double* Vw, const double* X, const double* UHB,
                                       const double* ell, const double* s2, const double* Bm, const double* M0,
                                       const double* xq, const double* jitter2, double* Mk, double* Bk, double* W,
                                       int Bt, int N, int n, int m, void* stream);
int bcbf_unicycle_control_step_rbfm52_f32(
    const float* Lop, const float* Vw, const float* X, const float* UHB, const float* ell, const float* s2,
    const float* Bm, const float* M0, const float* A, float* x, const float* plan, const float* dot_plan,
    const float* Kp, float clf_gamma, const float* centers, const float* radii, const float* tw, const float* gammas,
    float L_mean, const float* w, const float* r, const float* sign, const float* relax_mask, const float* rho,
    float* grad, float* cst, float* fhat, float* ghat, float* Mk, float* Bk, float* cones, int* cstatus,
    float* y, int* status, int* iters, float dt, float L_true, int Bt, int N, int Kob, int max_iters, int shared_gp,
    void* ev_start, void* ev_stop, void* stream);
int bcbf_unicycle_control_step_rbfm52_f64(
    const double* Lop, const double* Vw, const double* X, const double* UHB, const double* ell, const double* s2,
    const double* Bm, const double* M0, const double* A, double* x, const double* plan, const double* dot_plan,
    const double* Kp, double clf_gamma, const double* centers, const double* radii, const double* tw,
    const double* gammas, double L_mean, const double* w, const double* r, const double* sign,
    const double* relax_mask, const double* rho, double* grad, double* cst, double* fhat, double* ghat, double* Mk,
    double* Bk, double* cones, int* cstatus, double* y, int* status, int* iters, double dt, double L_true, int Bt,
    int N, int Kob, int max_iters, int shared_gp, void* ev_start, void* ev_stop, void* stream);

#pragma GCC visibility pop
#ifdef __cplusplus
}
#endif
#endif
```

Before: 12.59 million.

## Add mixed-precision two-phase interior-point SOCP solver with fp32 warm phase

```diff
diff --git a/bayesian_cbf_amd/_lib.py b/bayesian_cbf_amd/_lib.py
--- a/bayesian_cbf_amd/_lib.py
+++ b/bayesian_cbf_amd/_lib.py
@@ -109,6 +109,8 @@
     "bcbf_cbc_terms": [P, P, P, P, P, P, P, P, P, P, P, c_int, c_int, c_int, c_int, P],
     "bcbf_socp": [P, P, P, P, P, P, P, P, c_int, c_int, c_int, c_int, P],
     "bcbf_cbc_socp": [P] * 18 + [c_int, c_int, c_int, c_int, c_int, P],
+    "bcbf_cbc_socp_precision": [P] * 18 + [c_int, c_int, c_int, c_int, c_int, c_int, P],
+    "bcbf_unicycle_solve_step": [P] * 7 + ["T"] + [P] * 4 + ["T"] + [P] * 10 + ["T", "T", c_int, c_int, c_int, c_int, P],
     "bcbf_unicycle_constraints": [P, P, P, P, "T", P, P, P, P, "T", P, P, P, P, c_int, c_int, P],
     "bcbf_unicycle_step": [P, P, "T", "T", c_int, P],
     "bcbf_pendulum_plant_step": [P, P, "T", "T", "T", "T", c_int, P],
diff --git a/bayesian_cbf_amd/build.py b/bayesian_cbf_amd/build.py
--- a/bayesian_cbf_amd/build.py
+++ b/bayesian_cbf_amd/build.py
@@ -22,7 +22,8 @@
                "posterior_shared_reg.hip": ["-Rpass-analysis=kernel-resource-usage"],
                "posterior_step.hip": ["-Rpass-analysis=kernel-resource-usage"],
                "pendulum_qp.hip": ["-Rpass-analysis=kernel-resource-usage"],
-               "pendulum.hip": ["-Rpass-analysis=kernel-resource-usage"]}
+               "pendulum.hip": ["-Rpass-analysis=kernel-resource-usage"],
+               "socp_quad.hip": ["-Rpass-analysis=kernel-resource-usage"]}
 ZERO_SCRATCH_KERNELS = {"posterior_step.hip": [
     "posterior_step_kernel<float, 2, 4, 0, 1, false, 0,", "posterior_step_kernel<float, 3, 4, 0, 1, false, 0,",
     "posterior_step_kernel<double, 2, 4, 0, 1, false, 0,", "posterior_step_kernel<double, 3, 4, 0, 1, false, 0,",
@@ -30,7 +31,9 @@
     "posterior_step_kernel<float, 3, 4, 0, 1, false, 1, false, false>", "posterior_step_kernel<float, 3, 4, 0, 1, true, 0,",
     "posterior_step_kernel<double, 4, 4, 0, 1, false, 0,", "posterior_step_kernel<double, 3, 8, 0, 1, false, 0,"],
     "pendulum_qp.hip": ["pendulum_clf_cbf_rollout_kernel<float>", "pendulum_clf_cbf_rollout_kernel<double>"],
-    "pendulum.hip": ["pendulum_sampled_plant_kernel<double>"]}
+    "pendulum.hip": ["pendulum_sampled_plant_kernel<double>"],
+    "socp_quad.hip": ["socp_quad_kernel<float, 2, true, true, false, true>", "socp_quad_kernel<float, 2, true, true, false, false>",
+                      "socp_quad_kernel<float, 2, true, true, true, true>"]}
 SCRATCH_ALLOWANCE = {"posterior_step_kernel<float, 3, 4, 3, 1, false, 0,": 40}
 NO_SCRATCH = {"posterior_shared_reg.hip"}
 
diff --git a/bayesian_cbf_amd/csrc/control_step.hip b/bayesian_cbf_amd/csrc/control_step.hip
--- a/bayesian_cbf_amd/csrc/control_step.hip
+++ b/bayesian_cbf_amd/csrc/control_step.hip
@@ -5,7 +5,7 @@
 template <typename T>
 int launch_unicycle_socp(const T* Mk, const T* Bk, const T* A, const T* sign, const T* w, const T* r, const T* relax_mask,
                          const T* rho, T* cones, int* cstatus, T* y, int* status, int* iters, int Bt, int max_iters,
-                         const UnicycleTask<T>& task, void* stream);
+                         const UnicycleTask<T>& task, int all_fp64, void* stream);
 }
 
 #define BCBF_CTRL(T, SUF, NAME, QUERY, STEP)                                                                           \
@@ -32,7 +32,7 @@
         task.dt = dt; task.L_true = L_true; task.grad = grad; task.cst = cst; task.fhat = fhat; task.ghat = ghat;      \
         task.Kob = Kob;                                                                                                \
         return bcbf::launch_unicycle_socp<T>(Mk, Bk, A, sign, w, r, relax_mask, rho, cones, cstatus, y, status, iters, \
-                                             Bt, max_iters, task, stream);                                             \
+                                             Bt, max_iters, task, 0, stream);                                             \
     }
 #define BCBF_STEP_RBF(SUF) bcbf_posterior_step_##SUF(Lop, Vw, X, UHB, ell, s2, Bm, M0, x, nullptr, Mk, Bk, Bt, N, 3, 2, stream)
 #define BCBF_STEP_M52(SUF) bcbf_posterior_query_matern52_##SUF(Lop, Vw, X, UHB, ell, s2, Bm, M0, x, nullptr, Mk, Bk, nullptr, 0, Bt, N, 3, 2, stream)
@@ -72,7 +72,7 @@
         task.Kob = Kob; task.obs_x = obs_x; task.obs_uh = obs_uh; task.obs_y = obs_y; task.obs_ld = obs_ld;            \
         task.xq_next = xq_next; task.shift_invariant = flags & 1; task.advance_plan = (flags >> 1) & 1;                \
         return bcbf::launch_unicycle_socp<T>(Mk, Bk, A, sign, w, r, relax_mask, rho, cones, cstatus, y, status, iters, \
-                                             Bt, max_iters, task, stream);                                             \
+                                             Bt, max_iters, task, 0, stream);                                             \
     }
 BCBF_CTRL_OBS(float, f32)
 BCBF_CTRL_OBS(double, f64)
@@ -114,7 +114,7 @@
         task.xq_next = xq_next; task.shift_invariant = flags & 1; task.advance_plan = (flags >> 1) & 1;                \
         task.z = z; task.xdot_s = xdot_s; task.cbc_s = cbc_s;                                                          \
         return bcbf::launch_unicycle_socp<T>(Mk, Bk, A, sign, w, r, relax_mask, rho, cones, cstatus, y, status, iters, \
-                                             Bt, max_iters, task, stream);                                             \
+                                             Bt, max_iters, task, 0, stream);                                             \
     }
 BCBF_CTRL_SAMPLED(float, f32)
 BCBF_CTRL_SAMPLED(double, f64)
diff --git a/bayesian_cbf_amd/csrc/socp_quad.hip b/bayesian_cbf_amd/csrc/socp_quad.hip
--- a/bayesian_cbf_amd/csrc/socp_quad.hip
+++ b/bayesian_cbf_amd/csrc/socp_quad.hip
@@ -87,15 +87,22 @@
             out[a] = (a == 0 ? t : -t) * ib2;
         }
     }
-    __device__ inline void sinv(R* x) const {
-        R det = lam[0] * lam[0], lx = 0;
-#pragma unroll
-        for (int i = 1; i < D; ++i) { det -= lam[i] * lam[i]; lx += lam[i] * x[i]; }
-        const R y0 = qdv(lam[0] * x[0] - lx, det);
-        const R il0 = qdv(R(1), lam[0]);
+    struct LamTerms { R det, inrm, il0; };
+    __device__ inline LamTerms lam_terms() const {
+        LamTerms t;
+        t.det = jdet(lam);
+        t.inrm = qdv(R(1), qsq(t.det));
+        t.il0 = qdv(R(1), lam[0]);
+        return t;
+    }
+    __device__ inline void sinv(R* x, const LamTerms& lt) const {
+        R lx = 0;
+#pragma unroll
+        for (int i = 1; i < D; ++i) lx += lam[i] * x[i];
+        const R y0 = qdv(lam[0] * x[0] - lx, lt.det);
         x[0] = y0;
 #pragma unroll
-        for (int i = 1; i < D; ++i) x[i] = (x[i] - y0 * lam[i]) * il0;
+        for (int i = 1; i < D; ++i) x[i] = (x[i] - y0 * lam[i]) * lt.il0;
     }
     static __device__ inline void sprod(const R* x, const R* y, R* out) {
         R d = 0;
@@ -105,8 +112,8 @@
 #pragma unroll
         for (int i = 1; i < D; ++i) out[i] = x[0] * y[i] + y[0] * x[i];
     }
-    __device__ inline R scaled_max_step(const R* x) const {
-        const R nrm = qsq(jdet(lam)), inrm = qdv(R(1), nrm);
+    __device__ inline R scaled_max_step(const R* x, const LamTerms& lt) const {
+        const R inrm = lt.inrm;
         const R lb0 = lam[0] * inrm;
         R lx = 0;
 #pragma unroll
@@ -153,20 +160,25 @@
     y = y * (1.5 - 0.5 * d * y * y);
     return y;
 }
-template <int NV>
-__device__ inline bool chol3(double (*H)[NV]) {
+__device__ inline float rsqrt_d(float d) {
+    float y = __builtin_amdgcn_rsqf(d);
+    y = y * (1.5f - 0.5f * d * y * y);
+    return y;
+}
+template <int NV, typename F>
+__device__ inline bool chol3(F (*H)[NV]) {
     bool ok = true;
 #pragma unroll
     for (int j = 0; j < NV; ++j) {
-        double d = H[j][j];
+        F d = H[j][j];
 #pragma unroll
         for (int k = 0; k < NV; ++k) if (k < j) d -= H[j][k] * H[j][k];
-        if (!(d > 0.0)) { ok = false; d = 1.0; }
-        const double il = rsqrt_d(d);
+        if (!(d > F(0))) { ok = false; d = F(1); }
+        const F il = rsqrt_d(d);
         H[j][j] = il;
 #pragma unroll
         for (int i = 0; i < NV; ++i) if (i > j) {
-            double v = H[i][j];
+            F v = H[i][j];
 #pragma unroll
             for (int k = 0; k < NV; ++k) if (k < j) v -= H[i][k] * H[j][k];
             H[i][j] = v * il;
@@ -174,11 +186,11 @@
     }
     return ok;
 }
-template <int NV>
-__device__ inline void chol3_solve(const double (*H)[NV], double* b) {
+template <int NV, typename F>
+__device__ inline void chol3_solve(const F (*H)[NV], F* b) {
 #pragma unroll
     for (int i = 0; i < NV; ++i) {
-        double v = b[i];
+        F v = b[i];
 #pragma unroll
         for (int k = 0; k < NV; ++k) if (k < i) v -= H[i][k] * b[k];
         b[i] = v * H[i][i];
@@ -186,10 +198,221 @@
 #pragma unroll
     for (int ii = 0; ii < NV; ++ii) {
         const int i = NV - 1 - ii;
-        double v = b[i];
+        F v = b[i];
 #pragma unroll
         for (int k = 0; k < NV; ++k) if (k > i) v -= H[k][i] * b[k];
         b[i] = v * H[i][i];
+    }
+}
+
+template <typename R, int M_>
+struct QuadProgram {
+    static constexpr int NV = M_ + 1, D = M_ + 2;
+    R G[D][NV], h[D], Pd[NV], qv[NV], resx0, resz0, ideg;
+    template <typename S> __device__ inline void from(const QuadProgram<S, M_>& o) {
+#pragma unroll
+        for (int a = 0; a < D; ++a) {
+            h[a] = (R)o.h[a];
+#pragma unroll
+            for (int i = 0; i < NV; ++i) G[a][i] = (R)o.G[a][i];
+        }
+#pragma unroll
+        for (int i = 0; i < NV; ++i) { Pd[i] = (R)o.Pd[i]; qv[i] = (R)o.qv[i]; }
+        resx0 = (R)o.resx0; resz0 = (R)o.resz0; ideg = (R)o.ideg;
+    }
+};
+
+#ifndef BCBF_SOCP_HANDOVER
+#define BCBF_SOCP_HANDOVER 1e-2f
+#endif
+#ifndef BCBF_SOCP_A_CAP
+#define BCBF_SOCP_A_CAP 12
+#endif
+#ifndef BCBF_SOCP_A_FACTOR
+#define BCBF_SOCP_A_FACTOR double
+#endif
+constexpr int QUAD_A_HANDOVER = -1, QUAD_A_FAILED = -2;
+
+template <typename R, typename F, int M_, bool PHASE_A>
+__device__ inline int quad_iterate(const QuadProgram<R, M_>& p, ConeLane<R, M_ + 2>& cone, R (&x)[M_ + 1], const bool active,
+                                   int& it, const int it_end) {
+    constexpr int NV = M_ + 1, D = M_ + 2;
+    const bool act = active;
+    R xbest[NV], best = R(1e30);
+#pragma unroll
+    for (int i = 0; i < NV; ++i) xbest[i] = x[i];
+    int stall = 0, st_code = BCBF_SOCP_MAXITER;
+    F H[NV][NV];
+    for (; it <= it_end; ++it) {
+        const R ib2 = qdv(R(1), cone.beta2);
+        R gz[NV], rz[D], rzt[D];
+#pragma unroll
+        for (int i = 0; i < NV; ++i) {
+            R t = 0;
+#pragma unroll
+            for (int a = 0; a < D; ++a) t += p.G[a][i] * cone.z[a];
+            gz[i] = quad_sum(active ? t : R(0));
+        }
+        R f0 = 0, resx = 0, rz2 = 0, gp = 0;
+        R rx[NV];
+#pragma unroll
+        for (int i = 0; i < NV; ++i) {
+            const R px = p.Pd[i] * x[i];
+            f0 += x[i] * (R(0.5) * px + p.qv[i]);
+            rx[i] = px + p.qv[i] + gz[i];
+            resx += rx[i] * rx[i];
+        }
+#pragma unroll
+        for (int a = 0; a < D; ++a) {
+            R v = cone.s[a] - p.h[a];
+#pragma unroll
+            for (int i = 0; i < NV; ++i) v += p.G[a][i] * x[i];
+            rz[a] = v;
+            rz2 += v * v;
+            gp += cone.lam[a] * cone.lam[a];
+        }
+        cone.minv(rz, rzt, ib2);
+        R lrz = 0;
+#pragma unroll
+        for (int a = 0; a < D; ++a) lrz += cone.lam[a] * rzt[a];
+        resx = qsq(resx);
+        const R resz = qsq(quad_sum(active ? rz2 : R(0)));
+        const R gap = quad_sum(active ? gp : R(0));
+        lrz = quad_sum(active ? lrz : R(0));
+        const R pcost = f0, dcost = f0 + lrz - gap;
+        R relgap = R(1e30);
+        if (pcost < R(0)) relgap = qdv(gap, -pcost);
+        else if (dcost > R(0)) relgap = qdv(gap, dcost);
+        const R pres = qdv(resz, p.resz0), dres = qdv(resx, p.resx0);
+        R xmax = 0;
+#pragma unroll
+        for (int i = 0; i < NV; ++i) xmax = fmax(xmax, fabs(x[i]));
+        if constexpr (PHASE_A) {
+            if (!(gap + resx + resz < R(1e30)) || !(xmax < R(1e12)) || !(gap > R(0))) return QUAD_A_FAILED;
+        } else {
+            if (pres <= QTol<R>::feas() && dres <= QTol<R>::feas() && (gap <= QTol<R>::gap() || relgap <= QTol<R>::gap())) {
+                st_code = BCBF_SOCP_OPTIMAL;
+                break;
+            }
+        }
+        {
+            const R merit = fmax(fmax(pres, dres), fmin(gap, relgap));
+            stall = merit < R(0.9) * best ? 0 : stall + 1;
+            if (merit < best) {
+                best = merit;
+#pragma unroll
+                for (int i = 0; i < NV; ++i) xbest[i] = x[i];
+            }
+            if constexpr (PHASE_A) {
+                if (merit < R(BCBF_SOCP_HANDOVER) || stall >= 3) return QUAD_A_HANDOVER;
+            } else {
+                if (stall >= 3 && best <= QTol<R>::accept()) break;
+            }
+        }
+        {
+            R hz = 0, gzn = 0;
+#pragma unroll
+            for (int a = 0; a < D; ++a) hz += p.h[a] * cone.z[a];
+            hz = quad_sum(active ? hz : R(0));
+#pragma unroll
+            for (int i = 0; i < NV; ++i) gzn += gz[i] * gz[i];
+            if constexpr (PHASE_A) {
+                if (hz < R(0) && qsq(gzn) <= R(BCBF_SOCP_HANDOVER) * p.resx0 * (-hz)) return QUAD_A_HANDOVER;
+            } else {
+                if (hz < R(0) && qsq(gzn) <= QTol<R>::infeas() * p.resx0 * (-hz)) { st_code = BCBF_SOCP_DIVERGED; break; }
+            }
+        }
+        if constexpr (!PHASE_A)
+            if (!(gap + resx + resz < R(1e30)) || !(xmax < R(1e12))) { st_code = BCBF_SOCP_DIVERGED; break; }
+        if (it == it_end) break;
+
+        R Gt[D][NV];
+#pragma unroll
+        for (int i = 0; i < NV; ++i) {
+            R col[D], out[D];
+#pragma unroll
+            for (int a = 0; a < D; ++a) col[a] = p.G[a][i];
+            cone.minv(col, out, ib2);
+#pragma unroll
+            for (int a = 0; a < D; ++a) Gt[a][i] = out[a];
+        }
+#pragma unroll
+        for (int i = 0; i < NV; ++i)
+#pragma unroll
+            for (int j = 0; j < NV; ++j) if (j <= i) {
+                F v = F(0);
+#pragma unroll
+                for (int a = 0; a < D; ++a) v += (F)Gt[a][i] * (F)Gt[a][j];
+                H[i][j] = quad_sum(act ? v : F(0)) + (i == j ? (F)p.Pd[i] : F(0));
+            }
+        if (!chol3<NV>(H)) {
+            if constexpr (PHASE_A) return QUAD_A_FAILED;
+            st_code = BCBF_SOCP_DIVERGED;
+            break;
+        }
+
+        R lsq[D], corr[D], dx[NV], dst[D], dzt[D];
+        ConeLane<R, D>::sprod(cone.lam, cone.lam, lsq);
+#pragma unroll
+        for (int a = 0; a < D; ++a) corr[a] = R(0);
+        const typename ConeLane<R, D>::LamTerms lt = cone.lam_terms();
+        const R mu = gap * p.ideg;
+        R sigma = R(0), step = R(1);
+#pragma unroll
+        for (int pass = 0; pass < 2; ++pass) {
+            R c[D];
+#pragma unroll
+            for (int a = 0; a < D; ++a) c[a] = -lsq[a] - corr[a];
+            c[0] += sigma * mu;
+            cone.sinv(c, lt);
+            F rh3[NV];
+#pragma unroll
+            for (int i = 0; i < NV; ++i) {
+                F t = F(0);
+#pragma unroll
+                for (int a = 0; a < D; ++a) t += (F)Gt[a][i] * (F)(rzt[a] + c[a]);
+                rh3[i] = -(F)rx[i] - quad_sum(act ? t : F(0));
+            }
+            chol3_solve<NV>(H, rh3);
+#pragma unroll
+            for (int i = 0; i < NV; ++i) dx[i] = (R)rh3[i];
+#pragma unroll
+            for (int a = 0; a < D; ++a) {
+                R t = rzt[a];
+#pragma unroll
+                for (int i = 0; i < NV; ++i) t += Gt[a][i] * dx[i];
+                dzt[a] = t + c[a];
+                dst[a] = -t;
+            }
+            R dsdz = 0;
+            if (pass == 0) {
+                ConeLane<R, D>::sprod(dst, dzt, corr);
+#pragma unroll
+                for (int a = 0; a < D; ++a) dsdz += dst[a] * dzt[a];
+                dsdz = quad_sum(active ? dsdz : R(0));
+            }
+            const R tloc = active ? fmax(cone.scaled_max_step(dst, lt), cone.scaled_max_step(dzt, lt)) : R(-1e30);
+            const R tm = fmax(R(0), quad_max(tloc));
+            if (tm == R(0)) step = R(1);
+            else step = pass == 0 ? fmin(R(1), qdv(R(1), tm)) : fmin(R(1), qdv(R(0.99), tm));
+            if (pass == 0) {
+                const R sg = fmin(R(1), fmax(R(0), R(1) - step + qdv(dsdz, gap) * step * step));
+                sigma = sg * sg * sg;
+            }
+        }
+#pragma unroll
+        for (int i = 0; i < NV; ++i) x[i] += step * dx[i];
+        if (active) cone.advance(dst, dzt, step, ib2);
+    }
+    if constexpr (PHASE_A) {
+        return QUAD_A_HANDOVER;
+    } else {
+        if (st_code != BCBF_SOCP_OPTIMAL && best <= QTol<R>::accept()) {
+#pragma unroll
+            for (int i = 0; i < NV; ++i) x[i] = xbest[i];
+            st_code = BCBF_SOCP_OPTIMAL;
+        }
+        return st_code;
     }
 }
 
@@ -204,7 +427,7 @@
     return v;
 }
 
-template <typename T, int M_, bool FROM_TERMS, bool UNI, bool SAMPLED = false>
+template <typename T, int M_, bool FROM_TERMS, bool UNI, bool SAMPLED = false, bool MIXED = true>
 __global__ void __launch_bounds__(64)
 socp_quad_kernel(const T* __restrict__ w, const T* __restrict__ r, const T* __restrict__ cones_in,
                  const T* __restrict__ relax_mask, const T* __restrict__ rho,
@@ -229,7 +452,9 @@
     const int kk = active ? k : 0;
     [[maybe_unused]] SampledKeep<T, SAMPLED> keep;
 
-    R G[D][NV], h[D];
+    QuadProgram<R, M_> prog;
+    R (&G)[D][NV] = prog.G;
+    R (&h)[D] = prog.h;
     const R rh = (R)rho[bb];
     int bad = 0;
     {
@@ -419,7 +644,9 @@
     const bool act = active;
     const bool any_bad = quad_max((R)bad) > R(0);
 
-    R Pd[NV], qv[NV], x[NV];
+    R (&Pd)[NV] = prog.Pd;
+    R (&qv)[NV] = prog.qv;
+    R x[NV];
 #pragma unroll
     for (int i = 0; i < NV; ++i) {
         const R wi = (R)w[(size_t)bb * NV + i];
@@ -480,169 +707,58 @@
             for (int a = 0; a < D; ++a) { cone.s[a] = a == 0 ? R(1) : R(0); cone.z[a] = cone.s[a]; }
         }
     }
+    prog.resx0 = resx0; prog.resz0 = resz0; prog.ideg = qdv(R(1), (R)K);
+    int st_code = BCBF_SOCP_DIVERGED, it = 0;
+    [[maybe_unused]] int it_a = 0, fell_back = 0;
+    if constexpr (MIXED) {
+        if (okc) {
+            QuadProgram<float, M_> pf;
+            pf.from(prog);
+            ConeLane<float, D> ca;
+            float xa[NV];
+#pragma unroll
+            for (int i = 0; i < NV; ++i) xa[i] = (float)x[i];
+#pragma unroll
+            for (int a = 0; a < D; ++a) { ca.s[a] = (float)cone.s[a]; ca.z[a] = (float)cone.z[a]; }
+            ca.init_scaling();
+            const int cap = min((int)BCBF_SOCP_A_CAP, max_iters);
+            const int ra = quad_iterate<float, BCBF_SOCP_A_FACTOR, M_, true>(pf, ca, xa, active, it, cap);
+            if (ra == QUAD_A_HANDOVER && it > 0) {
+#pragma unroll
+                for (int i = 0; i < NV; ++i) x[i] = (R)xa[i];
+                R s2 = 0, z2 = 0, ns = 0, nz = 0;
+#pragma unroll
+                for (int a = 0; a < D; ++a) {
+                    cone.s[a] = (R)ca.s[a]; cone.z[a] = (R)ca.z[a];
+                    s2 += cone.s[a] * cone.s[a]; z2 += cone.z[a] * cone.z[a];
+                    if (a > 0) { ns += cone.s[a] * cone.s[a]; nz += cone.z[a] * cone.z[a]; }
+                }
+                const R nrms = fmax(qsq(quad_sum(active ? s2 : R(0))), R(1)), nrmz = fmax(qsq(quad_sum(active ? z2 : R(0))), R(1));
+                const R ts = quad_max(active ? qsq(ns) - cone.s[0] : R(-1e30));
+                const R tz = quad_max(active ? qsq(nz) - cone.z[0] : R(-1e30));
+                if (ts >= R(-1e-8) * nrms) cone.s[0] += R(1) + ts;
+                if (tz >= R(-1e-8) * nrmz) cone.z[0] += R(1) + tz;
+                if (!active) {
+#pragma unroll
+                    for (int a = 0; a < D; ++a) { cone.s[a] = a == 0 ? R(1) : R(0); cone.z[a] = cone.s[a]; }
+                }
+            }
+            it_a = it;
+            fell_back = ra == QUAD_A_FAILED;
+        }
+    }
     cone.init_scaling();
-
-    R xbest[NV], best = R(1e30);
-#pragma unroll
-    for (int i = 0; i < NV; ++i) xbest[i] = x[i];
-    int stall = 0, st_code = BCBF_SOCP_MAXITER, it = 0;
-    const R ideg = qdv(R(1), (R)K);
-    if (!okc) st_code = BCBF_SOCP_DIVERGED;
-
-    for (it = 0; it <= max_iters && okc; ++it) {
-        const R ib2 = qdv(R(1), cone.beta2);
-        R gz[NV], rz[D], rzt[D];
-#pragma unroll
-        for (int i = 0; i < NV; ++i) {
-            R t = 0;
-#pragma unroll
-            for (int a = 0; a < D; ++a) t += G[a][i] * cone.z[a];
-            gz[i] = quad_sum(active ? t : R(0));
-        }
-        R f0 = 0, resx = 0, rz2 = 0, gp = 0;
-        R rx[NV];
-#pragma unroll
-        for (int i = 0; i < NV; ++i) {
-            const R px = Pd[i] * x[i];
-            f0 += x[i] * (R(0.5) * px + qv[i]);
-            rx[i] = px + qv[i] + gz[i];
-            resx += rx[i] * rx[i];
-        }
-#pragma unroll
-        for (int a = 0; a < D; ++a) {
-            R v = cone.s[a] - h[a];
-#pragma unroll
-            for (int i = 0; i < NV; ++i) v += G[a][i] * x[i];
-            rz[a] = v;
-            rz2 += v * v;
-            gp += cone.lam[a] * cone.lam[a];
-        }
-        cone.minv(rz, rzt, ib2);
-        R lrz = 0;
-#pragma unroll
-        for (int a = 0; a < D; ++a) lrz += cone.lam[a] * rzt[a];
-        resx = qsq(resx);
-        const R resz = qsq(quad_sum(active ? rz2 : R(0)));
-        const R gap = quad_sum(active ? gp : R(0));
-        lrz = quad_sum(active ? lrz : R(0));
-        const R pcost = f0, dcost = f0 + lrz - gap;
-        R relgap = R(1e30);
-        if (pcost < R(0)) relgap = qdv(gap, -pcost);
-        else if (dcost > R(0)) relgap = qdv(gap, dcost);
-        const R pres = qdv(resz, resz0), dres = qdv(resx, resx0);
-        if (pres <= QTol<R>::feas() && dres <= QTol<R>::feas() && (gap <= QTol<R>::gap() || relgap <= QTol<R>::gap())) {
-            st_code = BCBF_SOCP_OPTIMAL;
-            break;
-        }
-        {
-            const R merit = fmax(fmax(pres, dres), fmin(gap, relgap));
-            stall = merit < R(0.9) * best ? 0 : stall + 1;
-            if (merit < best) {
-                best = merit;
-#pragma unroll
-                for (int i = 0; i < NV; ++i) xbest[i] = x[i];
-            }
-            if (stall >= 3 && best <= QTol<R>::accept()) break;
-        }
-        {
-            R hz = 0, gzn = 0;
-#pragma unroll
-            for (int a = 0; a < D; ++a) hz += h[a] * cone.z[a];
-            hz = quad_sum(active ? hz : R(0));
-#pragma unroll
-            for (int i = 0; i < NV; ++i) gzn += gz[i] * gz[i];
-            if (hz < R(0) && qsq(gzn) <= QTol<R>::infeas() * resx0 * (-hz)) { st_code = BCBF_SOCP_DIVERGED; break; }
-        }
-        R xmax = 0;
-#pragma unroll
-        for (int i = 0; i < NV; ++i) xmax = fmax(xmax, fabs(x[i]));
-        if (!(gap + resx + resz < R(1e30)) || !(xmax < R(1e12))) { st_code = BCBF_SOCP_DIVERGED; break; }
-        if (it == max_iters) break;
-
-        R Gt[D][NV];
-#pragma unroll
-        for (int i = 0; i < NV; ++i) {
-            R col[D], out[D];
-#pragma unroll
-            for (int a = 0; a < D; ++a) col[a] = G[a][i];
-            cone.minv(col, out, ib2);
-#pragma unroll
-            for (int a = 0; a < D; ++a) Gt[a][i] = out[a];
-        }
-#pragma unroll
-        for (int i = 0; i < NV; ++i)
-#pragma unroll
-            for (int j = 0; j < NV; ++j) if (j <= i) {
-                double v = 0.0;
-#pragma unroll
-                for (int a = 0; a < D; ++a) v += (double)Gt[a][i] * (double)Gt[a][j];
-                H[i][j] = quad_sum(act ? v : 0.0) + (i == j ? (double)Pd[i] : 0.0);
-            }
-        if (!chol3<NV>(H)) { st_code = BCBF_SOCP_DIVERGED; break; }
-
-        R lsq[D], corr[D], dx[NV], dst[D], dzt[D];
-        ConeLane<R, D>::sprod(cone.lam, cone.lam, lsq);
-#pragma unroll
-        for (int a = 0; a < D; ++a) corr[a] = R(0);
-        const R mu = gap * ideg;
-        R sigma = R(0), step = R(1);
-#pragma unroll
-        for (int pass = 0; pass < 2; ++pass) {
-            R c[D];
-#pragma unroll
-            for (int a = 0; a < D; ++a) c[a] = -lsq[a] - corr[a];
-            c[0] += sigma * mu;
-            cone.sinv(c);
-            double rh3[NV];
-#pragma unroll
-            for (int i = 0; i < NV; ++i) {
-                double t = 0.0;
-#pragma unroll
-                for (int a = 0; a < D; ++a) t += (double)Gt[a][i] * (double)(rzt[a] + c[a]);
-                rh3[i] = -(double)rx[i] - quad_sum(act ? t : 0.0);
-            }
-            chol3_solve<NV>(H, rh3);
-#pragma unroll
-            for (int i = 0; i < NV; ++i) dx[i] = (R)rh3[i];
-#pragma unroll
-            for (int a = 0; a < D; ++a) {
-                R t = rzt[a];
-#pragma unroll
-                for (int i = 0; i < NV; ++i) t += Gt[a][i] * dx[i];
-                dzt[a] = t + c[a];
-                dst[a] = -t;
-            }
-            R dsdz = 0;
-            if (pass == 0) {
-                ConeLane<R, D>::sprod(dst, dzt, corr);
-#pragma unroll
-                for (int a = 0; a < D; ++a) dsdz += dst[a] * dzt[a];
-                dsdz = quad_sum(active ? dsdz : R(0));
-            }
-            const R tloc = active ? fmax(cone.scaled_max_step(dst), cone.scaled_max_step(dzt)) : R(-1e30);
-            const R tm = fmax(R(0), quad_max(tloc));
-            if (tm == R(0)) step = R(1);
-            else step = pass == 0 ? fmin(R(1), qdv(R(1), tm)) : fmin(R(1), qdv(R(0.99), tm));
-            if (pass == 0) {
-                const R sg = fmin(R(1), fmax(R(0), R(1) - step + qdv(dsdz, gap) * step * step));
-                sigma = sg * sg * sg;
-            }
-        }
-#pragma unroll
-        for (int i = 0; i < NV; ++i) x[i] += step * dx[i];
-        if (active) cone.advance(dst, dzt, step, ib2);
-    }
-    if (st_code != BCBF_SOCP_OPTIMAL && best <= QTol<R>::accept()) {
-#pragma unroll
-        for (int i = 0; i < NV; ++i) x[i] = xbest[i];
-        st_code = BCBF_SOCP_OPTIMAL;
-    }
+    if (okc) st_code = quad_iterate<R, double, M_, false>(prog, cone, x, active, it, max_iters);
     if (any_bad) st_code = BCBF_SOCP_BADCONE;
     if (inst_ok && k == 0) {
 #pragma unroll
         for (int i = 0; i < NV; ++i) y[(size_t)b * NV + i] = (T)x[i];
         status[b] = st_code;
+#ifdef BCBF_SOCP_SWEEP_ITERS
+        if (iters) iters[b] = MIXED ? it + 1000 * it_a + 1000000 * fell_back : it;
+#else
         if (iters) iters[b] = it;
+#endif
         if (UNI && !SAMPLED && task.dt > T(0)) {
             T* xs = task.x + (size_t)b * 3;
             const T x0 = xs[0], x1 = xs[1], th = xs[2];
@@ -699,7 +815,7 @@
 static int launch_quad(const T* w, const T* r, const T* cones_in, const T* relax_mask, const T* rho, const T* Mk,
                        const T* Bk, const T* A, const T* grad, const T* cst, const T* sign, const T* fhat,
                        const T* ghat, int n, T* terms_out, T* cones_out, int* cstatus, T* y, int* status, int* iters,
-                       int Bt, int K, int m, int max_iters, void* stream, const UnicycleTask<T>* task = nullptr) {
+                       int Bt, int K, int m, int max_iters, int all_fp64, void* stream, const UnicycleTask<T>* task = nullptr) {
     if (Bt <= 0) return BCBF_OK;
     if (!w || !r || !relax_mask || !rho || !y || !status) return BCBF_EINVAL;
     if (K < 1 || K > 4 || m < 1 || m > BCBF_MAX_CTRL_DIM) return BCBF_EINVAL;
@@ -716,25 +832,31 @@
     const long lanes = (long)Bt * 4;
     dim3 grid((unsigned)((lanes + threads - 1) / threads)), block(threads);
     hipStream_t st = (hipStream_t)stream;
+    constexpr bool MIXED_IO = sizeof(T) == sizeof(float);
+#define BCBF_Q(MM, UNI_, SAMPLED_, MIXED_, TASK)                                                                        \
+    hipLaunchKernelGGL((socp_quad_kernel<T, MM, FROM_TERMS, UNI_, SAMPLED_, MIXED_>), grid, block, 0, st, w, r, cones_in,  \
+                       relax_mask, rho, Mk, Bk, A, grad, cst, sign, fhat, ghat, n, terms_out, cones_out, cstatus, y, status, \
+                       iters, Bt, K, max_iters, TASK)
+#define BCBF_QP(MM, UNI_, SAMPLED_, TASK)                                                                               \
+    do {                                                                                                                \
+        if constexpr (MIXED_IO) { if (!all_fp64) { BCBF_Q(MM, UNI_, SAMPLED_, true, TASK); break; } }                   \
+        BCBF_Q(MM, UNI_, SAMPLED_, false, TASK);                                                                        \
+    } while (0)
     if (FROM_TERMS && task != nullptr && task->z != nullptr) {
-        hipLaunchKernelGGL((socp_quad_kernel<T, 2, FROM_TERMS, FROM_TERMS, FROM_TERMS>), grid, block, 0, st, w, r, cones_in,
-                           relax_mask, rho, Mk, Bk, A, grad, cst, sign, fhat, ghat, n, terms_out, cones_out, cstatus, y, status,
-                           iters, Bt, K, max_iters, *task);
+        BCBF_QP(2, FROM_TERMS, FROM_TERMS, *task);
         return check_launch("unicycle_socp_sampled");
     }
     if (FROM_TERMS && task != nullptr) {
-        hipLaunchKernelGGL((socp_quad_kernel<T, 2, FROM_TERMS, FROM_TERMS>), grid, block, 0, st, w, r, cones_in, relax_mask,
-                           rho, Mk, Bk, A, grad, cst, sign, fhat, ghat, n, terms_out, cones_out, cstatus, y, status, iters,
-                           Bt, K, max_iters, *task);
+        BCBF_QP(2, FROM_TERMS, false, *task);
         return check_launch("unicycle_socp");
     }
-#define BCBF_Q(MM) hipLaunchKernelGGL((socp_quad_kernel<T, MM, FROM_TERMS, false>), grid, block, 0, st, w, r, cones_in, relax_mask, rho, Mk, Bk, A, grad, cst, sign, fhat, ghat, n, terms_out, cones_out, cstatus, y, status, iters, Bt, K, max_iters, UnicycleTask<T>{})
     switch (m) {
-        case 1: BCBF_Q(1); break;
-        case 2: BCBF_Q(2); break;
-        case 3: BCBF_Q(3); break;
+        case 1: BCBF_QP(1, false, false, UnicycleTask<T>{}); break;
+        case 2: BCBF_QP(2, false, false, UnicycleTask<T>{}); break;
+        case 3: BCBF_QP(3, false, false, UnicycleTask<T>{}); break;
         default: return BCBF_EINVAL;
     }
+#undef BCBF_QP
 #undef BCBF_Q
     return check_launch("socp_quad");
 }
@@ -742,16 +864,17 @@
 template <typename T>
 int launch_unicycle_socp(const T* Mk, const T* Bk, const T* A, const T* sign, const T* w, const T* r, const T* relax_mask,
                          const T* rho, T* cones, int* cstatus, T* y, int* status, int* iters, int Bt, int max_iters,
-                         const UnicycleTask<T>& task, void* stream) {
+                         const UnicycleTask<T>& task, int all_fp64, void* stream) {
     return launch_quad<T, true>(w, r, nullptr, relax_mask, rho, Mk, Bk, A, nullptr, nullptr, sign, nullptr, nullptr, 3,
-                                nullptr, cones, cstatus, y, status, iters, Bt, 1 + task.Kob, 2, max_iters, stream, &task);
+                                nullptr, cones, cstatus, y, status, iters, Bt, 1 + task.Kob, 2, max_iters, all_fp64, stream,
+                                &task);
 }
 template int launch_unicycle_socp<float>(const float*, const float*, const float*, const float*, const float*, const float*,
                                          const float*, const float*, float*, int*, float*, int*, int*, int, int,
-                                         const UnicycleTask<float>&, void*);
+                                         const UnicycleTask<float>&, int, void*);
 template int launch_unicycle_socp<double>(const double*, const double*, const double*, const double*, const double*,
                                           const double*, const double*, const double*, double*, int*, double*, int*, int*,
-                                          int, int, const UnicycleTask<double>&, void*);
+                                          int, int, const UnicycleTask<double>&, int, void*);
 
 }
 
@@ -760,26 +883,53 @@
                   float* y, int* status, int* iters, int Bt, int K, int m, int max_iters, void* stream) {
     return bcbf::launch_quad<float, false>(w, r, cones, relax_mask, rho, nullptr, nullptr, nullptr, nullptr, nullptr,
                                            nullptr, nullptr, nullptr, 0, nullptr, nullptr, nullptr, y, status, iters,
-                                           Bt, K, m, max_iters, stream);
+                                           Bt, K, m, max_iters, 0, stream);
 }
 int bcbf_socp_f64(const double* w, const double* r, const double* cones, const double* relax_mask, const double* rho,
                   double* y, int* status, int* iters, int Bt, int K, int m, int max_iters, void* stream) {
     return bcbf::launch_quad<double, false>(w, r, cones, relax_mask, rho, nullptr, nullptr, nullptr, nullptr, nullptr,
                                             nullptr, nullptr, nullptr, 0, nullptr, nullptr, nullptr, y, status, iters,
-                                            Bt, K, m, max_iters, stream);
+                                            Bt, K, m, max_iters, 0, stream);
 }
 int bcbf_cbc_socp_f32(const float* Mk, const float* Bk, const float* A, const float* grad, const float* cst,
                       const float* sign, const float* fhat, const float* ghat, const float* w, const float* r,
                       const float* relax_mask, const float* rho, float* terms, float* cones, int* cstatus,
                       float* y, int* status, int* iters, int Bt, int K, int n, int m, int max_iters, void* stream) {
     return bcbf::launch_quad<float, true>(w, r, nullptr, relax_mask, rho, Mk, Bk, A, grad, cst, sign, fhat, ghat, n,
-                                          terms, cones, cstatus, y, status, iters, Bt, K, m, max_iters, stream);
+                                          terms, cones, cstatus, y, status, iters, Bt, K, m, max_iters, 0, stream);
 }
 int bcbf_cbc_socp_f64(const double* Mk, const double* Bk, const double* A, const double* grad, const double* cst,
                       const double* sign, const double* fhat, const double* ghat, const double* w, const double* r,
                       const double* relax_mask, const double* rho, double* terms, double* cones, int* cstatus,
                       double* y, int* status, int* iters, int Bt, int K, int n, int m, int max_iters, void* stream) {
     return bcbf::launch_quad<double, true>(w, r, nullptr, relax_mask, rho, Mk, Bk, A, grad, cst, sign, fhat, ghat, n,
-                                           terms, cones, cstatus, y, status, iters, Bt, K, m, max_iters, stream);
-}
-}
+                                           terms, cones, cstatus, y, status, iters, Bt, K, m, max_iters, 0, stream);
+}
+
+#define BCBF_SOCP_PRECISION(T, SUF)                                                                                      \
+    int bcbf_cbc_socp_precision_##SUF(const T* Mk, const T* Bk, const T* A, const T* grad, const T* cst, const T* sign,  \
+                                      const T* fhat, const T* ghat, const T* w, const T* r, const T* relax_mask,         \
+                                      const T* rho, T* terms, T* cones, int* cstatus, T* y, int* status, int* iters,     \
+                                      int Bt, int K, int n, int m, int max_iters, int all_fp64, void* stream) {          \
+        return bcbf::launch_quad<T, true>(w, r, nullptr, relax_mask, rho, Mk, Bk, A, grad, cst, sign, fhat, ghat, n,     \
+                                          terms, cones, cstatus, y, status, iters, Bt, K, m, max_iters, all_fp64, stream); \
+    }                                                                                                                    \
+    int bcbf_unicycle_solve_step_##SUF(const T* Mk, const T* Bk, const T* A, T* x, const T* plan, const T* dot_plan,     \
+                                       const T* Kp, T clf_gamma, const T* centers, const T* radii, const T* tw,          \
+                                       const T* gammas, T L_mean, const T* w, const T* r, const T* sign,                 \
+                                       const T* relax_mask, const T* rho, T* cones, int* cstatus, T* y, int* status,     \
+                                       int* iters, T dt, T L_true, int Bt, int Kob, int max_iters, int all_fp64,         \
+                                       void* stream) {                                                                   \
+        if (Bt <= 0) return BCBF_OK;                                                                                     \
+        if (!x || Kob < 0 || Kob + 1 > BCBF_MAX_QUAD_CONSTRAINTS) return BCBF_EINVAL;                                    \
+        bcbf::UnicycleTask<T> task;                                                                                      \
+        task.x = x; task.plan = plan; task.dot_plan = dot_plan; task.Kp = Kp; task.centers = centers;                    \
+        task.radii = radii; task.tw = tw; task.gammas = gammas; task.clf_gamma = clf_gamma; task.L_mean = L_mean;        \
+        task.dt = dt; task.L_true = L_true; task.grad = nullptr; task.cst = nullptr; task.fhat = nullptr;                \
+        task.ghat = nullptr; task.Kob = Kob;                                                                             \
+        return bcbf::launch_unicycle_socp<T>(Mk, Bk, A, sign, w, r, relax_mask, rho, cones, cstatus, y, status, iters,   \
+                                             Bt, max_iters, task, all_fp64, stream);                                     \
+    }
+BCBF_SOCP_PRECISION(float, f32)
+BCBF_SOCP_PRECISION(double, f64)
+}
diff --git a/include/bcbf.h b/include/bcbf.h
--- a/include/bcbf.h
+++ b/include/bcbf.h
@@ -437,6 +437,29 @@
                       const double* sign, const double* fhat, const double* ghat, const double* w, const double* r,
                       const double* relax_mask, const double* rho, double* terms, double* cones, int* cstatus,
                       double* y, int* status, int* iters, int Bt, int K, int n, int m, int max_iters, void* stream);
+
+int bcbf_cbc_socp_precision_f32(const float* Mk, const float* Bk, const float* A, const float* grad, const float* cst,
+                                const float* sign, const float* fhat, const float* ghat, const float* w, const float* r,
+                                const float* relax_mask, const float* rho, float* terms, float* cones, int* cstatus,
+                                float* y, int* status, int* iters, int Bt, int K, int n, int m, int max_iters, int all_fp64,
+                                void* stream);
+int bcbf_cbc_socp_precision_f64(const double* Mk, const double* Bk, const double* A, const double* grad, const double* cst,
+                                const double* sign, const double* fhat, const double* ghat, const double* w, const double* r,
+                                const double* relax_mask, const double* rho, double* terms, double* cones, int* cstatus,
+                                double* y, int* status, int* iters, int Bt, int K, int n, int m, int max_iters, int all_fp64,
+                                void* stream);
+int bcbf_unicycle_solve_step_f32(const float* Mk, const float* Bk, const float* A, float* x, const float* plan,
+                                 const float* dot_plan, const float* Kp, float clf_gamma, const float* centers,
+                                 const float* radii, const float* tw, const float* gammas, float L_mean, const float* w,
+                                 const float* r, const float* sign, const float* relax_mask, const float* rho, float* cones,
+                                 int* cstatus, float* y, int* status, int* iters, float dt, float L_true, int Bt, int Kob,
+                                 int max_iters, int all_fp64, void* stream);
+int bcbf_unicycle_solve_step_f64(const double* Mk, const double* Bk, const double* A, double* x, const double* plan,
+                                 const double* dot_plan, const double* Kp, double clf_gamma, const double* centers,
+                                 const double* radii, const double* tw, const double* gammas, double L_mean, const double* w,
+                                 const double* r, const double* sign, const double* relax_mask, const double* rho, double* cones,
+                                 int* cstatus, double* y, int* status, int* iters, double dt, double L_true, int Bt, int Kob,
+                                 int max_iters, int all_fp64, void* stream);
 
 int bcbf_coneqp_f64(const double* P, const double* q, const double* G, const double* h,
                     int nv, int l, const int* qdims, int nq,
```

Measured after the change: 10.66 million. 15.4% lower.
